# Aster32/GAN-DANet

Measured on AMD Instinct MI355X. Metric: train samples/sec (G+D step) on 256x256 tiles, higher is better.
Workload: dtype bf16; 1 GPU; full G+D train step, 8ch 256x256 -> 1024x1024 tiles, batch 32/GPU (global 32), perceptual=on, SSIM evaluated, AdamW x2; survey_config=3, per_gpu_batch=32, global_batch=32, tile=256, parallelism=dp1

## Files before the change

gan-danet_amd/_lib.py:

```python
from __future__ import annotations

import ctypes as C
import os

HERE = os.path.dirname(os.path.abspath(__file__))
LIB_PATH = os.path.join(HERE, "lib", "libgandanet_hip.so")

PREC_FP32, PREC_BF16, PREC_X3 = 0, 1, 2
PAM_BWD_K64_ATOMIC, PAM_BWD_K64_PARTS, PAM_BWD_K32_PARTS, PAM_BWD_TWO_KERNEL = 0, 1, 2, 3
ACT_NONE, ACT_RELU, ACT_LEAKY02, ACT_SIGMOID = 0, 1, 2, 3
EVAL_F64, EVAL_SKIP_NAN = 1, 2
GUARD_SQNORM, GUARD_NORM, GUARD_COEF, GUARD_OK, GUARD_APPLIED, GUARD_SKIPPED, GUARD_RECORD = range(7)
GUARD_CHUNK = 65536
FILTER_F32, FILTER_F64 = 0, 1
EDGE_REFLECT, EDGE_INTERIOR = 0, 1
FILTER_MAX_RADIUS, SAVGOL_MAX_WINDOW = 64, 33
ZOOM_MIRROR, ZOOM_NEAREST = 0, 1
FREQ_MAX_BINS, FREQ_MAX_TABLE_BYTES = 33, 16 << 20
ZONE_MAX, ZONE_EDGE_CHUNK = 32, 512
STL_MAX_T = 2048

c_fp = C.c_void_p


# ... 100 lines not shown
    "gd_pam_wide_bwd": (_i, [_p, _p, _p, _p, _p, _p, _p, _i, _i, _i, _i, _i, _i, _i, _p, _p, _p, _p, _sz, _p]),
    "gd_pam_f32_fwd": (_i, [_p, _l, _p, _l, _p, _l, _i, _i, _i, _i, _i, _p, _p, _l, _p, _l, _p, _p, _p]),
    "gd_pam_f32_bwd": (_i, [_p, _l, _p, _l, _p, _l, _p, _l, _p, _p, _i, _i, _i, _i, _i, _p, _p, _p, _p]),
    "gd_pam_attn_stats": (_i, [_p, _l, _p, _l, _i, _i, _i, _i, _f, _p, _p, _p, _p]),
    "gd_pam_attn_received": (_i, [_p, _l, _p, _l, _p, _i, _i, _i, _i, _f, _p, _p]),
    "gd_pam_attn_rows": (_i, [_p, _l, _p, _l, _p, _i, _i, _i, _i, _i, _f, _p, _p, _p]),
    "gd_round_to_16": (_i, [_p, _p, _l, _f, _i, _p]),
    "gd_chan_dot": (_i, [_p, _l, _p, _l, _i, _i, _i, _p, _p, _p, _p]),
    "gd_pam_f16_scale": (_i, [_p, _l, _i, _i, _i, _p, _p, _p, _p, _p]),
    "gd_conv3x3_nhwc_pack": (_i, [_p, _i, _i, _i, _p, _sz, _p]),
    "gd_conv3x3_nhwc": (_i, [_p, _p, _p, _p, _p, _p, _i, _i, _i, _i, _i, _i, _i, _p]),
    "gd_conv3x3_nhwc_f32out": (_i, [_p, _p, _p, _p, _l, _i, _i, _i, _i, _i, _i, _p]),
    "gd_disc_stem_fwd": (_i, [_p, _i, _i, _i, _i, _p, _p, _i, _f, _p, _i, _p]),
    "gd_disc_stem_wgrad": (_i, [_p, _p, _i, _i, _i, _i, _i, _p, _p, _i, _p]),
    "gd_disc_stem_wgrad_ws": (_i, [_p, _p, _i, _i, _i, _i, _i, _p, _p, _i, _p, _p, _sz]),
    "gd_disc_stem_dgrad": (_i, [_p, _i, _i, _i, _i, _p, _i, _p, _i, _p]),
    "gd_conv3x3_nhwc_s2": (_i, [_p, _p, _p, _p, _i, _i, _i, _i, _i, _i, _f, _i, _p]),
    "gd_conv3x3_nhwc_s2_dgrad": (_i, [_p, _p, _p, _f, _p, _i, _i, _i, _i, _i, _i, _p]),
    "gd_nhwc_flatten_fwd": (_i, [_p, _i, _i, _i, _p, _i, _p]),
    "gd_nhwc_flatten_bwd": (_i, [_p, _p, _f, _i, _i, _i, _p, _i, _p]),
    "gd_nhwc_to_nchw16": (_i, [_p, _i, _i, _i, _p, _p, _i, _p]),
    "gd_nhwc_to_nchw16_ws": (_i, [_p, _i, _i, _i, _p, _p, _i, _p, _p, _sz]),
    "gd_nhwc_stem_fwd": (_i, [_p, _i, _i, _i, _i, _p, _p, _i, _i, _p, _i, _p]),
    "gd_nhwc_stem_bwd": (_i, [_p, _i, _i, _i, _i, _p, _i, _p, _i, _p]),
    "gd_nhwc_maxpool2_fwd": (_i, [_p, _i, _i, _i, _i, _p, _i, _p]),
    "gd_nhwc_maxpool2_bwd": (_i, [_p, _p, _i, _i, _i, _i, _i, _p, _i, _p]),
    "gd_nhwc_l1": (_i, [_p, _p, _l, _p, _i, _p, _i, _p]),
    "gd_nhwc_l1_grad": (_i, [_p, _p, _l, _p, _i, _p, _i, _p]),
    "gd_shift_sum9_fwd": (_i, [_p, _p, _p, _i, _i, _i, _p]),
    "gd_shift_sum9_bwd": (_i, [_p, _p, _i, _i, _i, _p]),
    "gd_combine_inputs": (_i, [_p, _i, _i, _i, _f, _p, _i, _i, _i, _f, _p, _i, _i, _i, _p]),
    "gd_hist_match_ws_bytes": (_sz, [_l, _l]),
    "gd_hist_match": (_i, [_p, _p, _i, _l, _l, C.c_double, _p, _p, _sz, _p]),
    "gd_eval_stats_ws_bytes": (_sz, [_l]),
    "gd_eval_stats": (_i, [_p, _p, _l, _l, _p, C.c_double, C.c_double, _i, _p, _p, _sz, _p]),
    "gd_masked_plane_mean_ws_bytes": (_sz, [_l, _l]),
    "gd_masked_plane_mean": (_i, [_p, _l, _l, _p, _p, _p, _p, _sz, _p]),
    "gd_ensemble_stats": (_i, [_p, _i, _l, _l, _i, _p, _p, _p]),
    "gd_eval_merge_host": (_i, [C.POINTER(C.c_double), _l, C.POINTER(C.c_double), C.POINTER(C.c_double)]),
    "gd_grad_sqnorm_ws_bytes": (_sz, [_l]),
    "gd_grad_sqnorm": (_i, [C.POINTER(_p), C.POINTER(_l), _i, _f, _i, _p, _p, _sz, _p]),
    "gd_guard_finalize": (_i, [_p, C.c_double, _i, _p]),
    "gd_adamw_guarded": (_i, [_p, _p, _p, _p, _p, _l, _p, _f, _f, _f, _f, _f, _f, _f, _p]),
    "gd_gaussian_weights_host": (_i, [C.c_double, C.c_double, C.POINTER(C.c_double), _i]),
    "gd_correlate1d_axis": (_i, [_p, _p, _i, _l, _l, _l, C.POINTER(C.c_double), _i, _i, _p]),
    "gd_savgol_edges_axis": (_i, [_p, _p, _i, _l, _l, _l, _p, _i, _p]),
    "gd_median_nd": (_i, [_p, _p, _i, C.POINTER(C.c_int64), C.POINTER(_i), _p]),
    "gd_fill_prepare": (_i, [_p, C.c_double, _p, _p, _i, _l, _p]),
    "gd_fill_ratio": (_i, [_p, _p, _p, C.c_double, _p, _i, _l, _p]),
    "gd_zoom_axis_ws_bytes": (_sz, [_l, _l, _l, _i, _i]),
    "gd_zoom_axis": (_i, [_p, _p, _i, _i, _l, _l, _l, _l, _i, _i, _p, _sz, _p]),
    "gd_spline_prefilter_axis": (_i, [_p, _p, _i, _l, _l, _l, _p]),
    "gd_restore_units": (_i, [_p, _i, _p, _i, _p, _l, _l, C.c_double, C.c_double, C.c_double, _p, _i, _p]),
    "gd_masked_plane_mean_f64_ws_bytes": (_sz, [_l, _l]),
    "gd_masked_plane_mean_f64": (_i, [_p, _l, _l, _p, _p, _p, _p, _sz, _p]),
    "gd_blend_region": (_i, [_p, _p, _p, _i, _i, _i, _i, _i, _i, _i, _p]),
    "gd_channel_moments_ws_bytes": (_sz, [_l, _l]),
    "gd_channel_moments": (_i, [_p, _i, _l, _l, _p, _p, _sz, _p]),
    "gd_scale_from_moments_host": (_i, [C.POINTER(C.c_double), _l, C.POINTER(C.c_double), C.POINTER(C.c_double),
                                        C.POINTER(C.c_double)]),
    "gd_channel_affine": (_i, [_p, _i, _p, _i, _l, _l, _p, _p, _i, _l, _l, _p]),
    "gd_freq_cos_table_host": (_i, [_l, _i, C.POINTER(C.c_double)]),
    "gd_freq_augment_axis": (_i, [_p, _p, _i, _l, _l, _l, _p, _i, _p, _p]),
    "gd_zone_rasterize": (_i, [_p, _l, C.POINTER(_l), _i, _p, _l, _p, _l, _p, _p]),
    "gd_zone_rasterize_host": (_i, [C.POINTER(C.c_double), _l, C.POINTER(_l), _i, C.POINTER(C.c_double), _l, C.POINTER(C.c_double), _l,
                                    C.POINTER(C.c_uint32)]),
    "gd_zone_mean_ws_bytes": (_sz, [_l, _l, _i]),
    "gd_zone_mean": (_i, [_p, _i, _l, _l, _p, _i, _p, _p, _p, _p, _sz, _p]),
    "gd_stl_decompose": (_i, [_p, _i, _l, _l, _i, _i, _i, _i, _i, _i, _i, _i, _i, _p, _p, _p, _p, _p]),
    "gd_stl_decompose_host": (_i, [_p, _i, _l, _l, _i, _i, _i, _i, _i, _i, _i, _i, _i, _p, _p, _p, _p]),
    "gd_augment_d4": (_i, [_p, _p, _i, _i, _i, _i, _p, _p, _f, _p]),
    "gd_bcast_mul": (_i, [_p, _p, _p, _i, _i, _l, _i, _p]),
    "gd_row_dot": (_i, [_p, _p, _p, _l, _l, _p]),
    "gd_chan_maxmean_fwd": (_i, [_p, _p, _p, _i, _i, _l, _p]),
    "gd_chan_maxmean_bwd": (_i, [_p, _p, _p, _i, _i, _l, _p]),
    "gd_comm_unique_id": (_i, [C.c_char_p]),
    "gd_comm_init": (_i, [_i, _i, C.c_char_p]),
    "gd_comm_world": (_i, []),
    "gd_allreduce": (_i, [_p, _sz, _i, _p]),
    "gd_reduce_scatter": (_i, [_p, _p, _sz, _i, _p]),
    "gd_allgather": (_i, [_p, _p, _sz, _i, _p]),
    "gd_comm_destroy": (_i, []),
    "gd_pack_bf16": (_i, [_p, _l, _i, _i, _i, _p, _f, _p, _i, _i, _p, _i, _i, _i, _i, _p]),
    "gd_pack_16": (_i, [_p, _l, _i, _i, _i, _p, _f, _p, _i, _i, _p, _i, _i, _i, _i, _i, _p]),
    "gd_pack_16_affine": (_i, [_p, _l, _i, _i, _i, _p, _p, _i, _p, _i, _i, _p, _i, _i, _i, _p]),
}

_lib = None


class GandanetError(RuntimeError):
    pass


def load() -> C.CDLL:
    global _lib
    if _lib is not None:
        return _lib
    if not os.path.exists(LIB_PATH):
        raise GandanetError(
            f"{LIB_PATH} is missing: the HIP extension is not built (run __graft_entry__.build()). "
            "There is no CPU fallback.")
    lib = C.CDLL(LIB_PATH)
    for name, (res, args) in SIGNATURES.items():
        fn = getattr(lib, name)
        fn.restype = res
        fn.argtypes = args
    if lib.gd_sizeof_conv_desc() != C.sizeof(ConvDesc) or lib.gd_sizeof_gemm_nt_desc() != C.sizeof(GemmNTDesc):
        raise GandanetError("descriptor struct layout differs between _lib.py and libgandanet_hip.so")
    _lib = lib
    return lib


def last_error() -> str:
    buf = C.create_string_buffer(512)
    load().gd_last_error(buf, 512)
    return buf.value.decode()


def check(rc: int, what: str = "") -> None:
    if rc != 0:
        raise GandanetError(f"{what or 'gandanet call'} failed (rc={rc}): {last_error()}")
```

gan-danet_amd/csrc/gemm_conv.hip:

```cpp
#include <stdlib.h>

#include <type_traits>

#include "common.h"
#include "tile_mma.h"
#include "../../include/gandanet.h"

namespace {

using gd::TILE_BK;
using gd::TILE_BN;
constexpr int BN = TILE_BN;
constexpr int BK = TILE_BK;

template <int BM, int MODE>
__global__ __launch_bounds__(256) void conv_nn_kernel(const gd_conv_desc d) {
    constexpr bool BF16 = MODE != gd::MODE_F32;
    constexpr bool X3 = MODE == gd::MODE_X3;
    using P = gd::TilePol<MODE>;
    using elem = typename P::elem;
    constexpr int LD = P::LD;
    constexpr int WAVES_N = gd::TileGeom<BM>::WAVES_N;
    constexpr int TM = gd::TileGeom<BM>::TM;
    constexpr int TN = gd::TileGeom<BM>::TN;
// ... 400 lines not shown
                            mma(acc[sb][i][j], fa[1][i], fb[0][j]);
                            mma(acc[sb][i][j], fa[0][i], fb[1][j]);
                        }
                        mma(acc[sb][i][j], fa[0][i], fb[0][j]);
                    }
            }
        }
        } else {
#pragma unroll
        for (int ks = 0; ks < BK / 16; ++ks) {
            bf16x8_t fa[TM];
#pragma unroll
            for (int i = 0; i < TM; ++i)
                fa[i] = *reinterpret_cast<const bf16x8_t*>(As + (wm * TM * 32 + i * 32 + r) * LDA + ks * 16 + 8 * h);
#pragma unroll
            for (int sb = 0; sb < NS; ++sb) {
                bf16x8_t fb[TN];
#pragma unroll
                for (int j = 0; j < TN; ++j) {
                    const unsigned short* p = Xs + sb * (BK * XLD) + (ks * 16 + 8 * h + tq) * XLD + (wn * TN + j) * 32 + 16 * tg + 4 * tp;
                    const s16x4_t lo = __builtin_amdgcn_ds_read_tr16_b64_v4i16((__attribute__((address_space(3))) s16x4_t*)p);
                    const s16x4_t hi = __builtin_amdgcn_ds_read_tr16_b64_v4i16(
                        (__attribute__((address_space(3))) s16x4_t*)(p + 4 * XLD));
                    fb[j] = bf16x8_t{lo.x, lo.y, lo.z, lo.w, hi.x, hi.y, hi.z, hi.w};
                }
#pragma unroll
                for (int i = 0; i < TM; ++i)
#pragma unroll
                    for (int j = 0; j < TN; ++j)
                        acc[sb][i][j] = __builtin_amdgcn_mfma_f32_32x32x16_bf16(
                            __builtin_bit_cast(gd::bf16x8_native_t, fa[i]), __builtin_bit_cast(gd::bf16x8_native_t, fb[j]),
                            acc[sb][i][j], 0, 0, 0);
            }
        }
        }
    };

    load_tile(0);
    store_tile();
    __syncthreads();
    for (int t = 0; t < T; ++t) {
        if (t + 1 < T) load_tile(t + 1);
        compute_tile();
        __syncthreads();
        if (t + 1 < T) {
            store_tile();
            __syncthreads();
        }
    }

    const float alpha = d.alpha ? *d.alpha : 1.f;
#pragma unroll
    for (int sb = 0; sb < NS; ++sb)
#pragma unroll
    for (int i = 0; i < TM; ++i)
#pragma unroll
        for (int j = 0; j < TN; ++j) {
            const int pn = n0 + sb * BN + wn * TN * 32 + j * 32 + r;
            if (pn >= HW) continue;
            float rsv[16], oldv[16];
#pragma unroll
            for (int e = 0; e < 16; ++e) {
                const int m = m0 + wm * TM * 32 + i * 32 + gd::acc_row(e, h);
                rsv[e] = (d.res && m < d.M) ? d.res[(long)b * d.res_bs + (long)m * HW + pn] : 0.f;
            }
#pragma unroll
            for (int e = 0; e < 16; ++e) {
                const int m = m0 + wm * TM * 32 + i * 32 + gd::acc_row(e, h);
                oldv[e] = (d.accumulate && m < d.M) ? reinterpret_cast<const float*>(d.y)[(long)b * d.y_bs + (long)m * HW + pn] : 0.f;
            }
#pragma unroll
            for (int e = 0; e < 16; ++e) {
                const int m = m0 + wm * TM * 32 + i * 32 + gd::acc_row(e, h);
                if (m >= d.M) continue;
                float v = acc[sb][i][j][e] * alpha + rsv[e];
                if (d.bias) v += d.bias[m];
                if (d.act == GD_ACT_RELU) v = fmaxf(v, 0.f);
                else if (d.act == GD_ACT_LEAKY02) v = v >= 0.f ? v : 0.2f * v;
                reinterpret_cast<float*>(d.y)[(long)b * d.y_bs + (long)m * HW + pn] = v + oldv[e];
            }
        }
}

template <int BM, bool X3 = false>
__global__ __launch_bounds__(256) void conv1x1_tr_plain_kernel(const gd_conv_desc d) {
    constexpr int LDA = BK + 8;
    constexpr int A_PL = BM * LDA, X_PL = BK * XLD;
    constexpr int WAVES_N = gd::TileGeom<BM>::WAVES_N;
    constexpr int TM = gd::TileGeom<BM>::TM;
    constexpr int TN = gd::TileGeom<BM>::TN;
    constexpr int KPT_A = BM / 8;
    __shared__ __attribute__((aligned(16))) unsigned short As[(X3 ? 2 : 1) * BM * LDA];
    __shared__ __attribute__((aligned(16))) unsigned short Xs[(X3 ? 2 : 1) * BK * XLD];

    const int tid = threadIdx.x, lane = tid & 63, wave = tid >> 6;
    const int r = lane & 31, h = lane >> 5;
    const int wm = wave / WAVES_N, wn = wave % WAVES_N;
    const int b = blockIdx.z, m0 = blockIdx.y * BM, n0 = blockIdx.x * BN;
    const int HW = d.Ho * d.Wo;

    const int am = tid % BM, akg = tid / BM;
    const bool a_row_ok = (m0 + am) < d.M;
    const float* a_row = d.a + (long)b * d.a_bs + (long)(m0 + am) * d.a_sm;

    const int xq = tid & 31, xr0 = tid >> 5;
    const float* x_img = d.x + (long)b * d.x_bs;
    const int pq = n0 + xq * 4;
    const bool q_full = pq + 3 < HW;

    f32x16_t acc[TM][TN];
#pragma unroll
    for (int i = 0; i < TM; ++i)
#pragma unroll
        for (int j = 0; j < TN; ++j)
#pragma unroll
            for (int e = 0; e < 16; ++e) acc[i][j][e] = 0.f;

    float ra[KPT_A];
    float4 rx[4];
    const int T = (d.Ck + BK - 1) / BK;
    auto load_tile = [&](int t) {
        const int c0 = t * BK;
#pragma unroll
        for (int i = 0; i < KPT_A; ++i) {
            const int c = c0 + akg * KPT_A + i;
            ra[i] = (a_row_ok && c < d.Ck) ? a_row[(long)c * d.a_sc] : 0.f;
        }
#pragma unroll
        for (int i = 0; i < 4; ++i) {
            const int c = c0 + xr0 + 8 * i;
            float4 v = make_float4(0.f, 0.f, 0.f, 0.f);
            if (c < d.Ck) {
                const float* p = x_img + (long)c * HW + pq;
                if (q_full) {
                    v = *reinterpret_cast<const float4*>(p);
                } else {
                    if (pq + 0 < HW) v.x = p[0];
                    if (pq + 1 < HW) v.y = p[1];
                    if (pq + 2 < HW) v.z = p[2];
                }
                if (d.in_scale) {
                    const float sc = d.in_scale[c], sh = d.in_shift[c];
                    v.x = fmaf(v.x, sc, sh); v.y = fmaf(v.y, sc, sh); v.z = fmaf(v.z, sc, sh); v.w = fmaf(v.w, sc, sh);
                    if (d.in_relu) {
                        v.x = fmaxf(v.x, 0.f); v.y = fmaxf(v.y, 0.f); v.z = fmaxf(v.z, 0.f); v.w = fmaxf(v.w, 0.f);
                    }
                    if (!q_full) {
                        if (pq + 0 >= HW) v.x = 0.f;
                        if (pq + 1 >= HW) v.y = 0.f;
                        if (pq + 2 >= HW) v.z = 0.f;
                        v.w = 0.f;
                    }
                }
            }
            rx[i] = v;
        }
    };
    auto store_tile = [&]() {
        unsigned short* ap = As + am * LDA + akg * KPT_A;
        if constexpr (X3) {
#pragma unroll
            for (int i = 0; i < KPT_A; i += 4) {
                uint2 whi, wlo;
                gd_split_bf2(ra[i + 0], ra[i + 1], whi.x, wlo.x);
                gd_split_bf2(ra[i + 2], ra[i + 3], whi.y, wlo.y);
                *reinterpret_cast<uint2*>(ap + i) = whi;
                *reinterpret_cast<uint2*>(ap + A_PL + i) = wlo;
            }
#pragma unroll
            for (int i = 0; i < 4; ++i) {
                uint2 whi, wlo;
                gd_split_bf2(rx[i].x, rx[i].y, whi.x, wlo.x);
                gd_split_bf2(rx[i].z, rx[i].w, whi.y, wlo.y);
                *reinterpret_cast<uint2*>(Xs + (xr0 + 8 * i) * XLD + xq * 4) = whi;
                *reinterpret_cast<uint2*>(Xs + X_PL + (xr0 + 8 * i) * XLD + xq * 4) = wlo;
            }
            return;
        }
        if constexpr (KPT_A >= 8) {
#pragma unroll
            for (int i = 0; i < KPT_A; i += 8) {
                uint4 w;
                w.x = gd_pack_bf2(ra[i + 0], ra[i + 1]);
                w.y = gd_pack_bf2(ra[i + 2], ra[i + 3]);
                w.z = gd_pack_bf2(ra[i + 4], ra[i + 5]);
                w.w = gd_pack_bf2(ra[i + 6], ra[i + 7]);
                *reinterpret_cast<uint4*>(ap + i) = w;
            }
        } else {
            uint2 w;
            w.x = gd_pack_bf2(ra[0], ra[1]);
            w.y = gd_pack_bf2(ra[2], ra[3]);
            *reinterpret_cast<uint2*>(ap) = w;
        }
#pragma unroll
        for (int i = 0; i < 4; ++i) {
            uint2 w;
            w.x = gd_pack_bf2(rx[i].x, rx[i].y);
            w.y = gd_pack_bf2(rx[i].z, rx[i].w);
            *reinterpret_cast<uint2*>(Xs + (xr0 + 8 * i) * XLD + xq * 4) = w;
        }
    };
    const int li = lane & 15, tq = li >> 2, tp = li & 3, tg = (lane >> 4) & 1;
    auto compute_tile = [&]() {
        if constexpr (X3) {
#pragma unroll
            for (int ks = 0; ks < BK / 16; ++ks) {
                bf16x8_t fa[2][TM], fb[2][TN];
#pragma unroll
                for (int pl = 0; pl < 2; ++pl) {
#pragma unroll
                    for (int i = 0; i < TM; ++i)
                        fa[pl][i] = *reinterpret_cast<const bf16x8_t*>(As + pl * A_PL + (wm * TM * 32 + i * 32 + r) * LDA + ks * 16 + 8 * h);
#pragma unroll
                    for (int j = 0; j < TN; ++j) {
                        const unsigned short* p = Xs + pl * X_PL + (ks * 16 + 8 * h + tq) * XLD + (wn * TN + j) * 32 + 16 * tg + 4 * tp;
// ... 63 lines not shown
            if (pn >= HW) continue;
            float rsv[16], oldv[16];
#pragma unroll
            for (int e = 0; e < 16; ++e) {
                const int m = m0 + wm * TM * 32 + i * 32 + gd::acc_row(e, h);
                rsv[e] = (d.res && m < d.M) ? d.res[(long)b * d.res_bs + (long)m * HW + pn] : 0.f;
            }
#pragma unroll
            for (int e = 0; e < 16; ++e) {
                const int m = m0 + wm * TM * 32 + i * 32 + gd::acc_row(e, h);
                oldv[e] = (d.accumulate && m < d.M) ? reinterpret_cast<const float*>(d.y)[(long)b * d.y_bs + (long)m * HW + pn] : 0.f;
            }
#pragma unroll
            for (int e = 0; e < 16; ++e) {
                const int m = m0 + wm * TM * 32 + i * 32 + gd::acc_row(e, h);
                if (m >= d.M) continue;
                float v = acc[i][j][e] * alpha + rsv[e];
                if (d.bias) v += d.bias[m];
                if (d.act == GD_ACT_RELU) v = fmaxf(v, 0.f);
                else if (d.act == GD_ACT_LEAKY02) v = v >= 0.f ? v : 0.2f * v;
                reinterpret_cast<float*>(d.y)[(long)b * d.y_bs + (long)m * HW + pn] = v + oldv[e];
            }
        }
}

static bool conv1x1_tr_eligible(const gd_conv_desc& d) {
    const long HW = (long)d.Ho * d.Wo;
    return d.ks == 1 && d.stride == 1 && d.pad == 0 && (d.precision == GD_PREC_BF16 || d.precision == GD_PREC_X3) && d.out_layout == 0 && !d.out_bf16 &&
           (d.Mstore == 0 || d.Mstore == d.M) && d.Hi == d.Ho && d.Wi == d.Wo && HW % 4 == 0 && d.x_bs % 4 == 0 &&
           ((uintptr_t)d.x % 16) == 0;
}

template <int BM>
int launch(const gd_conv_desc& d, hipStream_t s) {
    const int sstep = d.sub_step > 1 ? d.sub_step : 1;
    const long hs = (d.Ho - d.sub_oy + sstep - 1) / sstep, ws = (d.Wo - d.sub_ox + sstep - 1) / sstep;
    if (hs <= 0 || ws <= 0) return 0;
    dim3 grid(gd_cdiv(hs * ws, BN), gd_cdiv(d.Mstore, BM), d.B);
    if (d.precision == GD_PREC_BF16)
        hipLaunchKernelGGL((conv_nn_kernel<BM, gd::MODE_BF16>), grid, dim3(256), 0, s, d);
    else if (d.precision == GD_PREC_X3)
        hipLaunchKernelGGL((conv_nn_kernel<BM, gd::MODE_X3>), grid, dim3(256), 0, s, d);
    else
        hipLaunchKernelGGL((conv_nn_kernel<BM, gd::MODE_F32>), grid, dim3(256), 0, s, d);
    GD_LAUNCH_CHECK();
    return 0;
}

}

extern "C" int gd_conv2d(const gd_conv_desc* dp, void* stream) {
    GD_CHECK_ARG(dp != nullptr, "gd_conv2d: null descriptor");
    gd_conv_desc d = *dp;
    if (d.Mstore < d.M) d.Mstore = d.M;
    GD_CHECK_ARG(d.B > 0 && d.M > 0 && d.Ck > 0 && d.ks > 0 && d.stride > 0 && d.pad >= 0, "gd_conv2d: bad sizes");
    GD_CHECK_ARG(d.Hi > 0 && d.Wi > 0 && d.Ho > 0 && d.Wo > 0, "gd_conv2d: bad spatial sizes");
    GD_CHECK_ARG(d.a && d.x && d.y, "gd_conv2d: null tensor");
    GD_CHECK_ARG((d.in_scale == nullptr) == (d.in_shift == nullptr), "gd_conv2d: in_scale/in_shift must come together");
    GD_CHECK_ARG(d.precision == GD_PREC_FP32 || d.precision == GD_PREC_BF16 || d.precision == GD_PREC_X3, "gd_conv2d: bad precision");
    GD_CHECK_ARG(d.out_layout == 0 || (d.out_layout == 1 && d.ldo >= d.Mstore), "gd_conv2d: bad output layout");
    GD_CHECK_ARG(!(d.out_bf16 && d.accumulate), "gd_conv2d: accumulate needs an fp32 output");
    GD_CHECK_ARG((long)d.Ho * d.Wo < (1L << 31) && d.B <= 65535, "gd_conv2d: image too large for one launch");
    GD_CHECK_ARG(d.sub_step >= 0 && d.sub_oy >= 0 && d.sub_ox >= 0 && (d.sub_step > 1 || (d.sub_oy == 0 && d.sub_ox == 0)),
                 "gd_conv2d: bad output sub-lattice");
    if (!d.transposed) {
        GD_CHECK_ARG((d.Hi + 2 * d.pad - d.ks) / d.stride + 1 == d.Ho && (d.Wi + 2 * d.pad - d.ks) / d.stride + 1 == d.Wo,
                     "gd_conv2d: Ho/Wo do not match Hi/Wi, ks, stride, pad");
    } else {
        GD_CHECK_ARG((d.Ho + 2 * d.pad - d.ks) / d.stride + 1 == d.Hi && (d.Wo + 2 * d.pad - d.ks) / d.stride + 1 == d.Wi,
                     "gd_conv2d: transposed geometry mismatch");
    }
    hipStream_t s = (hipStream_t)stream;
    static const int tr_env = getenv("GD_CONV1X1_TR") ? atoi(getenv("GD_CONV1X1_TR")) : 1;
    if (tr_env && conv1x1_tr_eligible(d)) {
        const int bm = d.M <= 32 ? 32 : (d.M <= 64 || (d.M % 128 != 0 && d.M % 128 <= 64)) ? 64 : 128;
        static const int ns_env = getenv("GD_CONV1X1_NS") ? atoi(getenv("GD_CONV1X1_NS")) : 1;
        const long HWl = (long)d.Ho * d.Wo;
        int ns = (HWl * d.B >= (1L << 18) && d.precision == GD_PREC_BF16) ? ns_env : 1;
        if (bm == 128 && ns > 2) ns = 2;
        if (ns != 1 && ns != 2 && ns != 4) ns = 1;
        dim3 grid(gd_cdiv(HWl, BN * ns), gd_cdiv(d.M, bm), d.B);
#define GD_C1X1(BM_, NS_) hipLaunchKernelGGL((conv1x1_tr_kernel<BM_, NS_>), grid, dim3(256), 0, s, d)
        if (d.precision == GD_PREC_X3) {
            if (bm == 32) hipLaunchKernelGGL((conv1x1_tr_plain_kernel<32, true>), grid, dim3(256), 0, s, d);
            else if (bm == 64) hipLaunchKernelGGL((conv1x1_tr_plain_kernel<64, true>), grid, dim3(256), 0, s, d);
            else hipLaunchKernelGGL((conv1x1_tr_plain_kernel<128, true>), grid, dim3(256), 0, s, d);
        } else if (ns == 1) {
            if (bm == 32) hipLaunchKernelGGL((conv1x1_tr_plain_kernel<32>), grid, dim3(256), 0, s, d);
            else if (bm == 64) hipLaunchKernelGGL((conv1x1_tr_plain_kernel<64>), grid, dim3(256), 0, s, d);
            else hipLaunchKernelGGL((conv1x1_tr_plain_kernel<128>), grid, dim3(256), 0, s, d);
        } else
        if (bm == 32) { if (ns == 4) GD_C1X1(32, 4); else if (ns == 2) GD_C1X1(32, 2); else GD_C1X1(32, 1); }
        else if (bm == 64) { if (ns == 4) GD_C1X1(64, 4); else if (ns == 2) GD_C1X1(64, 2); else GD_C1X1(64, 1); }
        else { if (ns == 2) GD_C1X1(128, 2); else GD_C1X1(128, 1); }
#undef GD_C1X1
        GD_LAUNCH_CHECK();
        return 0;
    }
    auto run = [&](const gd_conv_desc& dd) -> int {
        if (dd.Mstore <= 32) return launch<32>(dd, s);
        if (dd.Mstore <= 64 || (dd.Mstore % 128 != 0 && dd.Mstore % 128 <= 64)) return launch<64>(dd, s);
        return launch<128>(dd, s);
    };
    if (d.transposed && d.stride > 1 && d.sub_step <= 1) {
        for (int py = 0; py < d.stride; ++py)
            for (int px = 0; px < d.stride; ++px) {
                gd_conv_desc dd = d;
                dd.sub_oy = py; dd.sub_ox = px; dd.sub_step = d.stride;
                const int rc = run(dd);
                if (rc) return rc;
            }
        return 0;
    }
    return run(d);
}
```

gan-danet_amd/csrc/gemm_nt.hip:

```cpp
#include "common.h"
#include "tile_mma.h"
#include "../../include/gandanet.h"

namespace {

using gd::TILE_BK;
using gd::TILE_BN;
constexpr int BN = TILE_BN;
constexpr int BK = TILE_BK;

__global__ void fill_zero_kernel(float* c, long c_bs, long ldc, int B, int M, int N) {
    const long total = (long)B * M * N;
    for (long i = (long)blockIdx.x * blockDim.x + threadIdx.x; i < total; i += (long)gridDim.x * blockDim.x) {
        const int n = (int)(i % N);
        const long t = i / N;
        const int m = (int)(t % M);
        const int b = (int)(t / M);
        c[(long)b * c_bs + (long)m * ldc + n] = 0.f;
    }
}

template <int BM, int MODE, bool VEC = false>
__global__ __launch_bounds__(256) void gemm_nt_kernel(const gd_gemm_nt_desc d, int ktiles, int tiles_per_split,
                                                      int splits, float* part) {
    constexpr bool BF16 = MODE != gd::MODE_F32;
    constexpr bool X3 = MODE == gd::MODE_X3;
    constexpr int A_PL = BM * gd::TilePol<MODE>::LD, B_PL = gd::TILE_BN * gd::TilePol<MODE>::LD;
    using P = gd::TilePol<MODE>;
    using elem = typename P::elem;
    constexpr int LD = P::LD;
    constexpr int WAVES_N = gd::TileGeom<BM>::WAVES_N;
    constexpr int TM = gd::TileGeom<BM>::TM;
    constexpr int TN = gd::TileGeom<BM>::TN;
    constexpr int RA = BM / 8;
    constexpr int RB = BN / 8;

    __shared__ __attribute__((aligned(16))) elem As[P::PLANES * BM * LD];
    __shared__ __attribute__((aligned(16))) elem Bs[P::PLANES * BN * LD];

    const int tid = threadIdx.x;
    const int lane = tid & 63, wave = tid >> 6;
    const int r = lane & 31, h = lane >> 5;
    const int wm = wave / WAVES_N, wn = wave % WAVES_N;
    const int b = blockIdx.z / splits;
    const int split = blockIdx.z - b * splits;
    const int m0 = blockIdx.y * BM;
    const int n0 = blockIdx.x * BN;
    const long K = (long)d.kseg * d.klen;

    const int kk = tid & 31;
    const int r0 = tid >> 5;

    const float* a_base = d.a + (long)b * d.a_bs;
    const float* b_base = d.bm + (long)b * d.b_bs;

    int rc_off[RB];
    int rc_dydx[RB];
    const int kss = d.ks * d.ks;
    if (d.im2col) {
#pragma unroll
        for (int i = 0; i < RB; ++i) {
            const int n = n0 + r0 + 8 * i;
            if (n < d.N) {
                const int c = n / kss, tap = n - c * kss;
                const int kh = tap / d.ks, kw = tap - kh * d.ks;
                rc_off[i] = c;
                rc_dydx[i] = (kh << 16) | kw;
            } else {
                rc_off[i] = 0;
                rc_dydx[i] = -1;
            }
        }
    }
    const long HiWi = (long)d.Hi * d.Wi;

    f32x16_t acc[TM][TN];
#pragma unroll
    for (int i = 0; i < TM; ++i)
#pragma unroll
        for (int j = 0; j < TN; ++j)
#pragma unroll
            for (int e = 0; e < 16; ++e) acc[i][j][e] = 0.f;

    float ra[RA], rb[RB];
    constexpr int RAV = BM / 32, RBV = BN / 32;
    float4 va[VEC ? RAV : 1], vb[VEC ? RBV : 1];
    const int kq = tid & 7, r0v = tid >> 3;

    auto load_tile_vec = [&](int t) {
        const long k = (long)t * BK + kq * 4;
        const bool k_ok = k < K;
        const int s = k_ok ? (int)(k / d.klen) : 0;
        const long kr = k_ok ? k - (long)s * d.klen : 0;
        const float* ap = a_base + (long)s * d.a_ss + kr;
        const float* bp = b_base + (long)s * d.b_ss + kr;
#pragma unroll
        for (int i = 0; i < RAV; ++i) {
            const int m = m0 + r0v + 32 * i;
            va[i] = (k_ok && m < d.M) ? *reinterpret_cast<const float4*>(ap + (long)m * d.lda) : make_float4(0, 0, 0, 0);
        }
#pragma unroll
        for (int i = 0; i < RBV; ++i) {
            const int n = n0 + r0v + 32 * i;
            vb[i] = (k_ok && n < d.N) ? *reinterpret_cast<const float4*>(bp + (long)n * d.ldb) : make_float4(0, 0, 0, 0);
        }
    };
    auto store_tile_vec = [&]() {
#pragma unroll
        for (int i = 0; i < RAV; ++i) {
            if constexpr (X3) {
                uint2 whi, wlo;
                gd_split_bf2(va[i].x, va[i].y, whi.x, wlo.x);
                gd_split_bf2(va[i].z, va[i].w, whi.y, wlo.y);
                *reinterpret_cast<uint2*>(As + (r0v + 32 * i) * LD + kq * 4) = whi;
                *reinterpret_cast<uint2*>(As + A_PL + (r0v + 32 * i) * LD + kq * 4) = wlo;
            } else if constexpr (BF16) {
                uint2 w;
                w.x = gd_pack_bf2(va[i].x, va[i].y);
                w.y = gd_pack_bf2(va[i].z, va[i].w);
                *reinterpret_cast<uint2*>(As + (r0v + 32 * i) * LD + kq * 4) = w;
            } else {
                float* p = reinterpret_cast<float*>(As) + (r0v + 32 * i) * LD + kq * 4;
                p[0] = va[i].x; p[1] = va[i].y; p[2] = va[i].z; p[3] = va[i].w;
            }
        }
#pragma unroll
        for (int i = 0; i < RBV; ++i) {
            if (d.in_scale) {
                const int n = n0 + r0v + 32 * i;
                if (n < d.N) {
// ... 71 lines not shown
    };

    auto store_tile = [&]() {
#pragma unroll
        for (int i = 0; i < RA; ++i) {
            if constexpr (X3) gd_split_bf(ra[i], As[(r0 + 8 * i) * LD + kk], As[A_PL + (r0 + 8 * i) * LD + kk]);
            else if constexpr (BF16) As[(r0 + 8 * i) * LD + kk] = gd_f2bf(ra[i]);
            else As[(r0 + 8 * i) * LD + kk] = ra[i];
        }
#pragma unroll
        for (int i = 0; i < RB; ++i) {
            if constexpr (X3) gd_split_bf(rb[i], Bs[(r0 + 8 * i) * LD + kk], Bs[B_PL + (r0 + 8 * i) * LD + kk]);
            else if constexpr (BF16) Bs[(r0 + 8 * i) * LD + kk] = gd_f2bf(rb[i]);
            else Bs[(r0 + 8 * i) * LD + kk] = rb[i];
        }
    };

    const int t_begin = split * tiles_per_split;
    const int t_end = min(ktiles, t_begin + tiles_per_split);
    if (t_begin >= t_end) return;

    if constexpr (VEC) {
        load_tile_vec(t_begin);
        store_tile_vec();
    } else {
        load_tile(t_begin);
        store_tile();
    }
    __syncthreads();
    for (int t = t_begin; t < t_end; ++t) {
        if (t + 1 < t_end) {
            if constexpr (VEC) load_tile_vec(t + 1);
            else load_tile(t + 1);
        }
        gd::tile_mma<BM, MODE>(As, Bs, wm, wn, r, h, acc);
        __syncthreads();
        if (t + 1 < t_end) {
            if constexpr (VEC) store_tile_vec();
            else store_tile();
            __syncthreads();
        }
    }

    const float alpha = d.alpha ? *d.alpha : 1.f;
    if (part) {
        float* pb = part + ((long)split * d.B + b) * d.M * d.N;
#pragma unroll
        for (int i = 0; i < TM; ++i) {
#pragma unroll
            for (int j = 0; j < TN; ++j) {
                const int n = n0 + wn * TN * 32 + j * 32 + r;
                if (n >= d.N) continue;
#pragma unroll
                for (int e = 0; e < 16; ++e) {
                    const int m = m0 + wm * TM * 32 + i * 32 + gd::acc_row(e, h);
                    if (m < d.M) pb[(long)m * d.N + n] = acc[i][j][e] * alpha;
                }
            }
        }
        return;
    }
    float* cb = d.c + (long)b * d.c_bs;
#pragma unroll
    for (int i = 0; i < TM; ++i) {
#pragma unroll
        for (int j = 0; j < TN; ++j) {
            const int n = n0 + wn * TN * 32 + j * 32 + r;
            if (n >= d.N) continue;
            const float bias = (d.bias && split == 0) ? d.bias[n] : 0.f;
#pragma unroll
            for (int e = 0; e < 16; ++e) {
                const int m = m0 + wm * TM * 32 + i * 32 + gd::acc_row(e, h);
                if (m >= d.M) continue;
                const float v = acc[i][j][e] * alpha + bias;
                float* cp = cb + (long)m * d.ldc + n;
                if (splits > 1) atomicAdd(cp, v);
                else if (d.accumulate) *cp += v;
                else *cp = v;
            }
        }
    }
}

template <int BM>
int launch(const gd_gemm_nt_desc& d, int ktiles, int tps, int splits, float* part, hipStream_t s) {
    if (splits > 1 && !d.accumulate && !part) {
        const long total = (long)d.B * d.M * d.N;
        const int blocks = (int)((total + 255) / 256 > 4096 ? 4096 : (total + 255) / 256);
        hipLaunchKernelGGL(fill_zero_kernel, dim3(blocks), dim3(256), 0, s, d.c, d.c_bs, d.ldc, d.B, d.M, d.N);
    }
    dim3 grid(gd_cdiv(d.N, BN), gd_cdiv(d.M, BM), d.B * splits);
    const bool vec = !d.im2col && d.klen % BK == 0 && d.lda % 4 == 0 && d.ldb % 4 == 0 &&
                     d.a_ss % 4 == 0 && d.b_ss % 4 == 0 && d.a_bs % 4 == 0 && d.b_bs % 4 == 0 &&
                     ((uintptr_t)d.a % 16) == 0 && ((uintptr_t)d.bm % 16) == 0;
    if (d.precision == GD_PREC_BF16) {
        if (vec) hipLaunchKernelGGL((gemm_nt_kernel<BM, gd::MODE_BF16, true>), grid, dim3(256), 0, s, d, ktiles, tps, splits, part);
        else hipLaunchKernelGGL((gemm_nt_kernel<BM, gd::MODE_BF16, false>), grid, dim3(256), 0, s, d, ktiles, tps, splits, part);
    } else if (d.precision == GD_PREC_X3) {
        if (vec) hipLaunchKernelGGL((gemm_nt_kernel<BM, gd::MODE_X3, true>), grid, dim3(256), 0, s, d, ktiles, tps, splits, part);
        else hipLaunchKernelGGL((gemm_nt_kernel<BM, gd::MODE_X3, false>), grid, dim3(256), 0, s, d, ktiles, tps, splits, part);
    } else {
        if (vec) hipLaunchKernelGGL((gemm_nt_kernel<BM, gd::MODE_F32, true>), grid, dim3(256), 0, s, d, ktiles, tps, splits, part);
        else hipLaunchKernelGGL((gemm_nt_kernel<BM, gd::MODE_F32, false>), grid, dim3(256), 0, s, d, ktiles, tps, splits, part);
    }
    GD_LAUNCH_CHECK();
    if (part) return gd_det_reduce_launch(part, splits, d.c, d.B, d.M, d.N, d.c_bs, d.ldc, d.bias, d.accumulate, s);
    return 0;
}

struct NtPlan { int ktiles, bm, tiles_per_split, splits, ordered; size_t ws_needed; };
int nt_plan(const gd_gemm_nt_desc& d, size_t ws_bytes, NtPlan* p) {
    GD_CHECK_ARG(d.B > 0 && d.M > 0 && d.N > 0 && d.kseg > 0 && d.klen > 0, "gd_gemm_nt: bad sizes");
    GD_CHECK_ARG((long)d.kseg * d.klen < (1L << 31), "gd_gemm_nt: reduction too long");
    GD_CHECK_ARG((d.in_scale == nullptr) == (d.in_shift == nullptr), "gd_gemm_nt: in_scale/in_shift must come together");
    GD_CHECK_ARG(d.precision == GD_PREC_FP32 || d.precision == GD_PREC_BF16 || d.precision == GD_PREC_X3, "gd_gemm_nt: bad precision");
    if (d.im2col) {
        GD_CHECK_ARG(d.ks > 0 && d.stride > 0 && d.pad >= 0 && d.Hi > 0 && d.Wi > 0 && d.Ho > 0 && d.Wo > 0,
                     "gd_gemm_nt: bad im2col geometry");
        GD_CHECK_ARG(d.klen == (long)d.Ho * d.Wo, "gd_gemm_nt: im2col needs klen == Ho*Wo");
        GD_CHECK_ARG(d.N % (d.ks * d.ks) == 0, "gd_gemm_nt: im2col needs N == C*ks*ks");
        GD_CHECK_ARG((d.Hi + 2 * d.pad - d.ks) / d.stride + 1 == d.Ho && (d.Wi + 2 * d.pad - d.ks) / d.stride + 1 == d.Wo,
                     "gd_gemm_nt: im2col Ho/Wo mismatch");
    }
    GD_CHECK_ARG((long)d.B * 4096 < 65535L * 64, "gd_gemm_nt: batch too large");
    const int ktiles = gd_cdiv((long)d.kseg * d.klen, BK);
    const int bm = d.M <= 32 ? 32 : (d.M <= 64 || (d.M % 128 != 0 && d.M % 128 <= 64)) ? 64 : 128;
    int splits = d.splits;
    if (splits <= 0) {
        const long tiles = (long)gd_cdiv(d.N, BN) * gd_cdiv(d.M, bm) * d.B;
        splits = (int)(2048 / tiles);
        if (splits < 1) splits = 1;
        if (splits > ktiles / 8) splits = ktiles / 8 > 0 ? ktiles / 8 : 1;
    }
    if (splits > ktiles) splits = ktiles;
    const bool det = gd_get_deterministic() != 0, ordered_mode = det && gd_get_det_reduce() == 1;
    if (det && !ordered_mode) splits = 1;
    if ((long)d.B * splits > 65535) splits = (int)(65535 / d.B);
    const size_t out_bytes = (size_t)d.B * d.M * d.N * sizeof(float);
    if (ordered_mode) {
        const size_t fit = ws_bytes / out_bytes;
        if ((size_t)splits > fit) splits = (int)fit;
        if (splits < 2) splits = 1;
    }
    const int tps = (ktiles + splits - 1) / splits;
    splits = (ktiles + tps - 1) / tps;
    p->ktiles = ktiles; p->bm = bm; p->tiles_per_split = tps; p->splits = splits;
    p->ordered = ordered_mode && splits > 1;
    p->ws_needed = p->ordered ? (size_t)splits * out_bytes : 0;
    return 0;
}

}

extern "C" int gd_gemm_nt_plan(const gd_gemm_nt_desc* dp, size_t ws_bytes, int* splits, size_t* ws_needed) {
    GD_CHECK_ARG(dp != nullptr, "gd_gemm_nt_plan: null descriptor");
    NtPlan p;
    if (nt_plan(*dp, ws_bytes, &p)) return -1;
    if (splits) *splits = p.splits;
    if (ws_needed) *ws_needed = p.ws_needed;
    return 0;
}

extern "C" int gd_gemm_nt_ws(const gd_gemm_nt_desc* dp, void* stream, void* ws, size_t ws_bytes) {
    GD_CHECK_ARG(dp != nullptr, "gd_gemm_nt: null descriptor");
    const gd_gemm_nt_desc& d = *dp;
    GD_CHECK_ARG(d.a && d.bm && d.c, "gd_gemm_nt: null tensor");
    GD_CHECK_ARG(((uintptr_t)ws % 16) == 0, "gd_gemm_nt: the workspace must be 16-byte aligned");
    NtPlan p;
    if (nt_plan(d, ws ? ws_bytes : 0, &p)) return -1;
    float* part = p.ordered ? (float*)ws : nullptr;
    hipStream_t s = (hipStream_t)stream;
    if (p.bm == 32) return launch<32>(d, p.ktiles, p.tiles_per_split, p.splits, part, s);
    if (p.bm == 64) return launch<64>(d, p.ktiles, p.tiles_per_split, p.splits, part, s);
    return launch<128>(d, p.ktiles, p.tiles_per_split, p.splits, part, s);
}

extern "C" int gd_gemm_nt(const gd_gemm_nt_desc* dp, void* stream) { return gd_gemm_nt_ws(dp, stream, nullptr, 0); }
```

gan-danet_amd/csrc/pointwise.hip:

```cpp
#include "common.h"
#include "../../include/gandanet.h"

#include <math.h>

namespace {

constexpr int RED_BLOCKS = 1024;

static inline int grid_for(long n, int per_block = 256 * 4) {
    long g = (n + per_block - 1) / per_block;
    if (g < 1) g = 1;
    if (g > 8192) g = 8192;
    return (int)g;
}

__device__ __forceinline__ float act_f(float v, int act) {
    if (act == GD_ACT_RELU) return fmaxf(v, 0.f);
    if (act == GD_ACT_LEAKY02) return v >= 0.f ? v : 0.2f * v;
    if (act == GD_ACT_SIGMOID) return 1.f / (1.f + __expf(-v));
    return v;
}

__global__ void act_fwd_kernel(const float* __restrict__ x, float* __restrict__ y, long n, int act) {
    for (long i = (long)blockIdx.x * blockDim.x + threadIdx.x; i < n; i += (long)gridDim.x * blockDim.x)
// ... 377 lines not shown
        for (long j = threadIdx.x; j < n; j += 256) s = fmaf(ap[j], bp[j], s);
        s = gd_block_sum(s, red);
        if (threadIdx.x == 0) out[row] = s;
    }
}
__global__ void chan_maxmean_fwd_kernel(const float* __restrict__ x, float* __restrict__ y, int* __restrict__ idx, int C,
                                        long HW, long total) {
    for (long i = (long)blockIdx.x * blockDim.x + threadIdx.x; i < total; i += (long)gridDim.x * blockDim.x) {
        const long b = i / HW, p = i - b * HW;
        const float* xp = x + b * C * HW + p;
        float mx = xp[0], sum = xp[0];
        int am = 0;
        for (int c = 1; c < C; ++c) {
            const float v = xp[(long)c * HW];
            sum += v;
            if (v > mx) { mx = v; am = c; }
        }
        y[b * 2 * HW + p] = mx;
        y[b * 2 * HW + HW + p] = sum / (float)C;
        idx[i] = am;
    }
}
__global__ void chan_maxmean_bwd_kernel(const float* __restrict__ dy, const int* __restrict__ idx, float* __restrict__ dx,
                                        int C, long HW, long total) {
    const float inv_c = 1.f / (float)C;
    for (long i = (long)blockIdx.x * blockDim.x + threadIdx.x; i < total; i += (long)gridDim.x * blockDim.x) {
        const long bc = i / HW, p = i - bc * HW;
        const long b = bc / C;
        const int c = (int)(bc - b * C);
        const float gmax = dy[b * 2 * HW + p], gmean = dy[b * 2 * HW + HW + p];
        dx[i] = gmean * inv_c + (idx[b * HW + p] == c ? gmax : 0.f);
    }
}

__global__ __launch_bounds__(256) void chan_dot_kernel(const float* __restrict__ a, long a_bs, const float* __restrict__ o,
                                                      long o_bs, int C, int N, const float* __restrict__ gamma,
                                                      float* __restrict__ draw, float* __restrict__ delta) {
    const int b = blockIdx.y;
    const int i = blockIdx.x * 256 + threadIdx.x;
    if (i >= N) return;
    const float* ap = a + (long)b * a_bs + i;
    const float* op = o + (long)b * o_bs + i;
    float s = 0.f;
    for (int c = 0; c < C; ++c) s = fmaf(ap[(long)c * N], op[(long)c * N], s);
    draw[(long)b * N + i] = s;
    delta[(long)b * N + i] = s * (*gamma);
}

__global__ __launch_bounds__(256) void absmax_kernel(const float* __restrict__ a, long a_bs, long chw, float* __restrict__ ws) {
    __shared__ float red[8];
    const float* ap = a + (long)blockIdx.y * a_bs;
    float m = 0.f;
    for (long i = (long)blockIdx.x * 256 + threadIdx.x; i < chw; i += (long)gridDim.x * 256) {
        const float v = fabsf(ap[i]);
        m = v > m ? v : m;
    }
    m = gd_block_max(m, red);
    if (threadIdx.x == 0) ws[blockIdx.y * gridDim.x + blockIdx.x] = m;
}
__global__ __launch_bounds__(256) void f16_scale_kernel(const float* __restrict__ ws, int nparts, const float* __restrict__ gamma,
                                                       float* __restrict__ delta, long n, float* __restrict__ scales) {
    __shared__ float red[8];
    __shared__ float s_up;
    float m = 0.f;
    for (int i = threadIdx.x; i < nparts; i += 256) m = fmaxf(m, ws[i]);
    m = gd_block_max(m, red);
    if (threadIdx.x == 0) {
        const float g = *gamma;
        const float t = m * fabsf(g);
        int e = 0;
        if (t > 0.f && t < 3.0e38f) frexpf(t, &e);
        e = e > 100 ? 100 : (e < -100 ? -100 : e);
        s_up = ldexpf(1.f, -e);
        if (blockIdx.x == 0) {
            scales[0] = g * s_up;
            scales[1] = ldexpf(1.f, e);
        }
    }
    __syncthreads();
    const float up = s_up;
    for (long i = (long)blockIdx.x * 256 + threadIdx.x; i < n; i += (long)gridDim.x * 256) delta[i] *= up;
}

__global__ __launch_bounds__(256) void bce_kernel(const float* __restrict__ z, long n, float label, float inv_n,
                                                 float* __restrict__ dz, float* __restrict__ ws) {
    __shared__ float red[8];
    float s = 0.f;
    for (long i = (long)blockIdx.x * 256 + threadIdx.x; i < n; i += (long)gridDim.x * 256) {
        const float v = z[i];
        s += fmaxf(v, 0.f) - v * label + log1pf(expf(-fabsf(v)));
        if (dz) dz[i] = (1.f / (1.f + expf(-v)) - label) * inv_n;
    }
    s = gd_block_sum(s, red);
    if (threadIdx.x == 0) ws[blockIdx.x] = s;
}
__global__ __launch_bounds__(256) void bce_target_kernel(const float* __restrict__ z, const float* __restrict__ t, long n,
                                                        float inv_n, float* __restrict__ dz, float* __restrict__ dt,
                                                        float* __restrict__ ws) {
    __shared__ float red[8];
    float s = 0.f;
    for (long i = (long)blockIdx.x * 256 + threadIdx.x; i < n; i += (long)gridDim.x * 256) {
        const float v = z[i], y = t[i];
        s += fmaxf(v, 0.f) - v * y + log1pf(expf(-fabsf(v)));
        if (dz) dz[i] = (1.f / (1.f + expf(-v)) - y) * inv_n;
        if (dt) dt[i] = -v * inv_n;
    }
    s = gd_block_sum(s, red);
    if (threadIdx.x == 0) ws[blockIdx.x] = s;
}
__global__ void leaky_fwd_kernel(const float* __restrict__ x, float* __restrict__ y, long n, float slope) {
    for (long i = (long)blockIdx.x * blockDim.x + threadIdx.x; i < n; i += (long)gridDim.x * blockDim.x) {
        const float v = x[i];
        y[i] = v >= 0.f ? v : slope * v;
    }
}
__global__ void leaky_bwd_kernel(const float* __restrict__ x, const float* __restrict__ dy, float* __restrict__ dx, long n,
                                 float slope) {
    for (long i = (long)blockIdx.x * blockDim.x + threadIdx.x; i < n; i += (long)gridDim.x * blockDim.x)
        dx[i] = x[i] >= 0.f ? dy[i] : slope * dy[i];
}
template <bool L1>
__global__ __launch_bounds__(256) void diff_loss_kernel(const float* __restrict__ a, const float* __restrict__ b, long n,
                                                       float inv_n, float* __restrict__ da, float* __restrict__ ws) {
    __shared__ float red[8];
    float s = 0.f;
    for (long i = (long)blockIdx.x * 256 + threadIdx.x; i < n; i += (long)gridDim.x * 256) {
        const float dv = a[i] - b[i];
        if (L1) {
            s += fabsf(dv);
            if (da) da[i] = dv > 0.f ? inv_n : (dv < 0.f ? -inv_n : 0.f);
        } else {
            s = fmaf(dv, dv, s);
            if (da) da[i] = 2.f * dv * inv_n;
        }
    }
    s = gd_block_sum(s, red);
    if (threadIdx.x == 0) ws[blockIdx.x] = s;
}
__global__ __launch_bounds__(256) void tv_kernel(const float* __restrict__ x, long planes, int H, int W, float kh, float kw,
                                                float* __restrict__ dx, float* __restrict__ ws_h, float* __restrict__ ws_w) {
    __shared__ float red[8];
    const long total = planes * H * W;
    float sh = 0.f, sw = 0.f;
    for (long i = (long)blockIdx.x * 256 + threadIdx.x; i < total; i += (long)gridDim.x * 256) {
        const int xx = (int)(i % W);
        const int yy = (int)((i / W) % H);
        const float v = x[i];
        float g = 0.f;
        if (yy + 1 < H) { const float d = x[i + W] - v; sh = fmaf(d, d, sh); g -= 2.f * kh * d; }
        if (yy > 0) { const float d = v - x[i - W]; g += 2.f * kh * d; }
        if (xx + 1 < W) { const float d = x[i + 1] - v; sw = fmaf(d, d, sw); g -= 2.f * kw * d; }
        if (xx > 0) { const float d = v - x[i - 1]; g += 2.f * kw * d; }
        if (dx) dx[i] = g;
    }
    sh = gd_block_sum(sh, red);
    sw = gd_block_sum(sw, red);
    if (threadIdx.x == 0) { ws_h[blockIdx.x] = sh; ws_w[blockIdx.x] = sw; }
}
__global__ __launch_bounds__(256) void tv_final_kernel(const float* __restrict__ ws_h, const float* __restrict__ ws_w,
                                                      int nparts, float kh, float kw, float* __restrict__ out) {
    __shared__ double redd[8];
    double a = 0, b = 0;
    for (int i = threadIdx.x; i < nparts; i += 256) { a += ws_h[i]; b += ws_w[i]; }
    a = gd_wave_sum_d(a);
    b = gd_wave_sum_d(b);
    if ((threadIdx.x & 63) == 0) { redd[threadIdx.x >> 6] = a; redd[4 + (threadIdx.x >> 6)] = b; }
// ... 283 lines not shown
    GD_LAUNCH_CHECK();
    return 0;
}
extern "C" int gd_pack_16_split(const float* s, long s_bs, int B, int R, int Cc, const float* row_scale, const float* row_shift,
                                int relu, void* plain, long p_bs, int ldp, long p_cs, int p_ncopy, int p_pattern, void* tr,
                                long t_bs, int ldt, long t_cs, int t_ncopy, int t_pattern, void* stream) {
    return gd_pack_16_split_masked(s, s_bs, B, R, Cc, row_scale, row_shift, relu, plain, p_bs, ldp, p_cs, p_ncopy, p_pattern, tr,
                                   t_bs, ldt, t_cs, t_ncopy, t_pattern, nullptr, 0, stream);
}
extern "C" int gd_split3_weights(const float* w, long A, long Bn, long Cn, float* out, void* stream) {
    GD_CHECK_ARG(w && out && A > 0 && Bn > 0 && Cn > 0, "gd_split3_weights: bad arguments");
    const long total = A * Bn * Cn;
    hipLaunchKernelGGL(split3_weights_kernel, dim3(grid_for(total) > 4096 ? 4096 : grid_for(total)), dim3(256), 0, GD_S, w, A, Bn, Cn, out);
    GD_LAUNCH_CHECK();
    return 0;
}
extern "C" int gd_pack_bf16(const float* s, long s_bs, int B, int R, int Cc, const float* scale_dev, float scale_imm,
                            void* plain, int Rp_plain, int ld_plain, void* transposed, int Ccp_t, int ld_t, int perm16,
                            int ones_row, void* stream) {
    return gd_pack_16(s, s_bs, B, R, Cc, scale_dev, scale_imm, plain, Rp_plain, ld_plain, transposed, Ccp_t, ld_t, perm16,
                      ones_row, 0, stream);
}
extern "C" int gd_augment_d4(const float* src, float* dst, int B, int C, int H, int W, const int* ops, const float* noise,
                             float noise_scale, void* stream) {
    GD_CHECK_ARG(src && dst && ops && src != dst && B > 0 && C > 0 && H > 0 && W > 0, "gd_augment_d4: bad arguments");
    const long total = (long)B * C * H * W;
    hipLaunchKernelGGL(augment_d4_kernel, dim3(grid_for(total)), dim3(256), 0, GD_S, src, dst, C, H, W, ops, noise,
                       noise_scale, total);
    GD_LAUNCH_CHECK();
    return 0;
}
extern "C" int gd_bcast_mul(const float* x, const float* att, float* y, int B, int C, long HW, int mode, void* stream) {
    GD_CHECK_ARG(x && att && y && B > 0 && C > 0 && HW > 0 && (mode == 0 || mode == 1), "gd_bcast_mul: bad arguments");
    const long total = (long)B * C * HW;
    hipLaunchKernelGGL(bcast_mul_kernel, dim3(grid_for(total)), dim3(256), 0, GD_S, x, att, y, C, HW, mode, total);
    GD_LAUNCH_CHECK();
    return 0;
}
extern "C" int gd_row_dot(const float* a, const float* b, float* out, long rows, long n, void* stream) {
    GD_CHECK_ARG(a && b && out && rows > 0 && n > 0, "gd_row_dot: bad arguments");
    hipLaunchKernelGGL(row_dot_kernel, dim3((unsigned)(rows < 8192 ? rows : 8192)), dim3(256), 0, GD_S, a, b, out, rows, n);
    GD_LAUNCH_CHECK();
    return 0;
}
extern "C" int gd_chan_maxmean_fwd(const float* x, float* y, int* idx, int B, int C, long HW, void* stream) {
    GD_CHECK_ARG(x && y && idx && B > 0 && C > 0 && HW > 0, "gd_chan_maxmean_fwd: bad arguments");
    const long total = (long)B * HW;
    hipLaunchKernelGGL(chan_maxmean_fwd_kernel, dim3(grid_for(total, 256)), dim3(256), 0, GD_S, x, y, idx, C, HW, total);
    GD_LAUNCH_CHECK();
    return 0;
}
extern "C" int gd_chan_maxmean_bwd(const float* dy, const int* idx, float* dx, int B, int C, long HW, void* stream) {
    GD_CHECK_ARG(dy && idx && dx && B > 0 && C > 0 && HW > 0, "gd_chan_maxmean_bwd: bad arguments");
    const long total = (long)B * C * HW;
    hipLaunchKernelGGL(chan_maxmean_bwd_kernel, dim3(grid_for(total)), dim3(256), 0, GD_S, dy, idx, dx, C, HW, total);
    GD_LAUNCH_CHECK();
    return 0;
}
extern "C" int gd_chan_dot(const float* a, long a_bs, const float* o, long o_bs, int B, int C, int N, const float* gamma,
                           float* d_raw, float* delta, void* stream) {
    GD_CHECK_ARG(a && o && gamma && d_raw && delta && B > 0 && B <= 65535 && C > 0 && N > 0, "gd_chan_dot: bad arguments");
    hipLaunchKernelGGL(chan_dot_kernel, dim3(gd_cdiv(N, 256), B), dim3(256), 0, GD_S, a, a_bs, o, o_bs, C, N, gamma, d_raw,
                       delta);
    GD_LAUNCH_CHECK();
    return 0;
}

extern "C" int gd_pam_f16_scale(const float* dout, long dout_bs, int B, int C, int N, const float* gamma, float* delta,
                                float* scales, float* ws, void* stream) {
    GD_CHECK_ARG(dout && gamma && delta && scales && ws && B > 0 && B <= 65535 && C > 0 && N > 0, "gd_pam_f16_scale: bad arguments");
    const long chw = (long)C * N;
    int g = grid_for(chw);
    g = g > RED_BLOCKS / B ? RED_BLOCKS / B : g;
    g = g < 1 ? 1 : g;
    GD_CHECK_ARG((long)g * B <= RED_BLOCKS, "gd_pam_f16_scale: batch larger than the reduction workspace (1024 parts)");
    hipLaunchKernelGGL(absmax_kernel, dim3(g, B), dim3(256), 0, GD_S, dout, dout_bs, chw, ws);
    const long n = (long)B * N;
    hipLaunchKernelGGL(f16_scale_kernel, dim3(grid_for(n) > 256 ? 256 : grid_for(n)), dim3(256), 0, GD_S, ws, g * B, gamma, delta, n,
                       scales);
    GD_LAUNCH_CHECK();
    return 0;
}

extern "C" int gd_bce_logits(const float* z, long n, float label, float* out, float* dz, float* ws, void* stream) {
    GD_CHECK_ARG(z && out && ws && n > 0, "gd_bce_logits: bad arguments");
    const int g = grid_for(n) > RED_BLOCKS ? RED_BLOCKS : grid_for(n);
    hipLaunchKernelGGL(bce_kernel, dim3(g), dim3(256), 0, GD_S, z, n, label, 1.f / (float)n, dz, ws);
    hipLaunchKernelGGL(reduce_final_kernel, dim3(1), dim3(256), 0, GD_S, ws, g, 1.f / (float)n, out, 0);
    GD_LAUNCH_CHECK();
    return 0;
}
extern "C" int gd_bce_logits_target(const float* z, const float* t, long n, float* out, float* dz, float* dt, float* ws,
                                    void* stream) {
    GD_CHECK_ARG(z && t && out && ws && n > 0, "gd_bce_logits_target: bad arguments");
    const int g = grid_for(n) > RED_BLOCKS ? RED_BLOCKS : grid_for(n);
    hipLaunchKernelGGL(bce_target_kernel, dim3(g), dim3(256), 0, GD_S, z, t, n, 1.f / (float)n, dz, dt, ws);
    hipLaunchKernelGGL(reduce_final_kernel, dim3(1), dim3(256), 0, GD_S, ws, g, 1.f / (float)n, out, 0);
    GD_LAUNCH_CHECK();
    return 0;
}
extern "C" int gd_leaky_fwd(const float* x, float* y, long n, float slope, void* stream) {
    GD_CHECK_ARG(x && y && n > 0, "gd_leaky_fwd: bad arguments");
    hipLaunchKernelGGL(leaky_fwd_kernel, dim3(grid_for(n)), dim3(256), 0, GD_S, x, y, n, slope);
    GD_LAUNCH_CHECK();
    return 0;
}
extern "C" int gd_leaky_bwd(const float* x, const float* dy, float* dx, long n, float slope, void* stream) {
    GD_CHECK_ARG(x && dy && dx && n > 0, "gd_leaky_bwd: bad arguments");
    hipLaunchKernelGGL(leaky_bwd_kernel, dim3(grid_for(n)), dim3(256), 0, GD_S, x, dy, dx, n, slope);
    GD_LAUNCH_CHECK();
    return 0;
}
extern "C" int gd_mse(const float* a, const float* b, long n, float* out, float* da, float* ws, void* stream) {
    GD_CHECK_ARG(a && b && out && ws && n > 0, "gd_mse: bad arguments");
    const int g = grid_for(n) > RED_BLOCKS ? RED_BLOCKS : grid_for(n);
    hipLaunchKernelGGL((diff_loss_kernel<false>), dim3(g), dim3(256), 0, GD_S, a, b, n, 1.f / (float)n, da, ws);
    hipLaunchKernelGGL(reduce_final_kernel, dim3(1), dim3(256), 0, GD_S, ws, g, 1.f / (float)n, out, 0);
    GD_LAUNCH_CHECK();
    return 0;
}
extern "C" int gd_l1(const float* a, const float* b, long n, float* out, float* da, float* ws, void* stream) {
    GD_CHECK_ARG(a && b && out && ws && n > 0, "gd_l1: bad arguments");
    const int g = grid_for(n) > RED_BLOCKS ? RED_BLOCKS : grid_for(n);
    hipLaunchKernelGGL((diff_loss_kernel<true>), dim3(g), dim3(256), 0, GD_S, a, b, n, 1.f / (float)n, da, ws);
    hipLaunchKernelGGL(reduce_final_kernel, dim3(1), dim3(256), 0, GD_S, ws, g, 1.f / (float)n, out, 0);
    GD_LAUNCH_CHECK();
    return 0;
}
extern "C" int gd_tv(const float* x, int B, int C, int H, int W, float weight, float* out, float* dx, float* ws,
                     void* stream) {
    GD_CHECK_ARG(x && out && ws && B > 0 && C > 0 && H > 1 && W > 1, "gd_tv: bad arguments");
    const long planes = (long)B * C;
    const double count_h = (double)planes * (H - 1) * W, count_w = (double)planes * H * (W - 1);
    const float kh = (float)(weight * 2.0 / count_h / B), kw = (float)(weight * 2.0 / count_w / B);
    const long n = planes * H * W;
    const int g = grid_for(n) > RED_BLOCKS ? RED_BLOCKS : grid_for(n);
    hipLaunchKernelGGL(tv_kernel, dim3(g), dim3(256), 0, GD_S, x, planes, H, W, kh, kw, dx, ws, ws + RED_BLOCKS);
    hipLaunchKernelGGL(tv_final_kernel, dim3(1), dim3(256), 0, GD_S, ws, ws + RED_BLOCKS, g, kh, kw, out);
    GD_LAUNCH_CHECK();
    return 0;
}
static int ssim_window(int window, SsimWin* win) {
    if (!(window > 0 && window <= 15 && (window & 1))) return -1;
    win->n = window;
    float tmp[16], sum = 0.f;
    for (int i = 0; i < window; ++i) {
        const float d = (float)(i - window / 2);
        tmp[i] = expf(-(d * d) / (2.f * 1.5f * 1.5f));
        sum += tmp[i];
    }
    for (int i = 0; i < 16; ++i) win->g[i] = i < window ? tmp[i] / sum : 0.f;
    return 0;
}
static int ssim_gx(int H, int W, int BC) {
    int gx = (int)(((long)H * W + 255) / 256);
    if (gx > 64) gx = 64;
    while ((long)gx * BC > 2048 && gx > 1) gx >>= 1;
    return gx;
}
extern "C" int gd_ssim(const float* a, const float* b, int BC, int H, int W, int window, float* out, float* ws,
                       void* stream) {
    GD_CHECK_ARG(a && b && out && ws && BC > 0 && H > 0 && W > 0, "gd_ssim: bad arguments");
    SsimWin win;
    GD_CHECK_ARG(ssim_window(window, &win) == 0, "gd_ssim: window must be odd and <= 15");
    const int gx = ssim_gx(H, W, BC);
    GD_CHECK_ARG((long)gx * BC <= 2048 && BC <= 65535, "gd_ssim: too many planes for the workspace");
// ... 51 lines not shown
```

gan-danet_amd/kern.py:

```python
from __future__ import annotations

import ctypes as C
import math
import os
from typing import Optional, Tuple

import torch

from . import _lib as L

Tensor = torch.Tensor


def _stream() -> int:
    return torch.cuda.current_stream().cuda_stream


def _ptr(t: Optional[Tensor]):
    return None if t is None else t.data_ptr()


def _chk(t: Tensor, name: str = "tensor", dtype=torch.float32) -> None:
    if not t.is_cuda:
        raise L.GandanetError(f"{name}: expected a GPU tensor (there is no CPU fallback in the product path)")
# ... 9 lines not shown


def _bview(t: Tensor, name: str = "tensor") -> int:
    _chk(t, name)
    if t.dim() == 4:
        b, c, h, w = t.shape
        ok = t.stride(3) == 1 and t.stride(2) == w and t.stride(1) == h * w
        inner = c * h * w
    elif t.dim() == 3:
        b, c, n = t.shape
        ok = t.stride(2) == 1 and t.stride(1) == n
        inner = c * n
    else:
        raise L.GandanetError(f"{name}: expected a 3-D or 4-D tensor")
    if not ok:
        raise L.GandanetError(f"{name}: per-image block must be dense, got strides {t.stride()}")
    bs = t.stride(0) if b > 1 else inner
    if b > 1 and bs < inner:
        raise L.GandanetError(f"{name}: overlapping batch stride")
    return bs


def lib():
    return L.load()


WGRAD_X_NHWC = os.environ.get("GD_WGRAD_X_NHWC", "1") != "0"
USE_CONV3X3_FAST = True


PROFILE_ON = False
PROFILE_CONV = os.environ.get("GD_PROFILE_CONV", "0") == "1"
PROFILE: list = []


class _Bracket:

    def __init__(self, name: str, flops: float, nbytes: float = 0.0):
        self.name, self.flops, self.nbytes = name, flops, nbytes

    def __enter__(self):
        if PROFILE_ON:
            self.e0 = torch.cuda.Event(enable_timing=True)
            self.e1 = torch.cuda.Event(enable_timing=True)
            self.e0.record()
        return self

    def __exit__(self, *exc):
        if PROFILE_ON:
            self.e1.record()
            PROFILE.append((self.name, self.e0, self.e1, self.flops, self.nbytes))
        return False


class _ConvBracket(_Bracket):

    def __init__(self, kind, k, stride, cin, cout, ho, wo, b):
        super().__init__(f"conv_{kind}_k{k}s{stride}_{cin}->{cout}@{ho}x{wo}", 2.0 * k * k * cin * cout * ho * wo * b)

    def __enter__(self):
        return super().__enter__() if PROFILE_CONV else self

    def __exit__(self, *exc):
        return super().__exit__(*exc) if PROFILE_CONV else False


def profile_summary():
    torch.cuda.synchronize()
    agg = {}
    for name, e0, e1, fl, nb in PROFILE:
        a = agg.setdefault(name, [0, 0.0, 0.0, 0.0])
        a[0] += 1
        a[1] += e0.elapsed_time(e1)
        a[2] += fl
        a[3] += nb
    return {k: (v[0], v[1] / v[0], v[2] / v[0], v[3] / v[0]) for k, v in agg.items()}


def conv_nn(*, B: int, M: int, Ck: int, ks: int, stride: int, pad: int, transposed: bool, Hi: int, Wi: int,
            Ho: int, Wo: int, a: Tensor, a_bs: int, a_sm: int, a_sc: int, a_st: int, x: Tensor, x_bs: int,
            y: Tensor, y_bs: int, precision: int, Mstore: int = 0, in_scale: Optional[Tensor] = None,
            in_shift: Optional[Tensor] = None, in_relu: bool = False, out_layout: int = 0, out_bf16: bool = False,
            ldo: int = 0, alpha: Optional[Tensor] = None, bias: Optional[Tensor] = None,
            res: Optional[Tensor] = None, res_bs: int = 0, act: int = 0, accumulate: bool = False) -> None:
    d = L.ConvDesc()
    d.B, d.M, d.Mstore, d.Ck, d.ks, d.stride, d.pad = B, M, max(M, Mstore), Ck, ks, stride, pad
    d.transposed = int(transposed)
    d.Hi, d.Wi, d.Ho, d.Wo = Hi, Wi, Ho, Wo
    d.a, d.a_bs, d.a_sm, d.a_sc, d.a_st = _ptr(a), a_bs, a_sm, a_sc, a_st
    d.x, d.x_bs = _ptr(x), x_bs
    d.in_scale, d.in_shift, d.in_relu = _ptr(in_scale), _ptr(in_shift), int(in_relu)
    d.y, d.y_bs = _ptr(y), y_bs
    d.out_layout, d.out_bf16, d.ldo = out_layout, int(out_bf16), ldo
    d.alpha, d.bias, d.res, d.res_bs = _ptr(alpha), _ptr(bias), _ptr(res), res_bs
    d.act, d.accumulate, d.precision = act, int(accumulate), precision
    if USE_CONV3X3_FAST and lib().gd_conv3x3_eligible(C.byref(d)):
        nbytes = int(lib().gd_conv3x3_ws_bytes(M, Ck))
        ws = torch.empty(nbytes // 2, device=x.device, dtype=torch.bfloat16)
        L.check(lib().gd_conv3x3(C.byref(d), _ptr(ws), nbytes, _stream()), "gd_conv3x3")
        return
    L.check(lib().gd_conv2d(C.byref(d), _stream()), "gd_conv2d")


def conv_out_size(h: int, k: int, stride: int, pad: int) -> int:
    return (h + 2 * pad - k) // stride + 1


def conv2d_fwd(x: Tensor, w: Tensor, bias: Optional[Tensor], stride: int, pad: int, precision: int, *,
               act: int = 0, out: Optional[Tensor] = None, in_scale=None, in_shift=None, in_relu=False,
               accumulate: bool = False) -> Tensor:
    xbs = _bview(x, "conv input")
    _dense(w, "conv weight")
    B, Cin, Hi, Wi = x.shape
    Cout, Cin_w, k, k2 = w.shape
    if Cin_w != Cin or k != k2:
        raise L.GandanetError(f"conv2d: weight {tuple(w.shape)} does not match input {tuple(x.shape)}")
    Ho, Wo = conv_out_size(Hi, k, stride, pad), conv_out_size(Wi, k, stride, pad)
    if out is None:
        out = torch.empty(B, Cout, Ho, Wo, device=x.device, dtype=torch.float32)
    elif tuple(out.shape) != (B, Cout, Ho, Wo):
        raise L.GandanetError("conv2d: bad out shape")
    with _ConvBracket("fwd", k, stride, Cin, Cout, Ho, Wo, B):
        conv_nn(B=B, M=Cout, Ck=Cin, ks=k, stride=stride, pad=pad, transposed=False, Hi=Hi, Wi=Wi, Ho=Ho, Wo=Wo,
                a=w, a_bs=0, a_sm=Cin * k * k, a_sc=k * k, a_st=1, x=x, x_bs=xbs, y=out, y_bs=_bview(out, "conv out"),
                precision=precision, in_scale=in_scale, in_shift=in_shift, in_relu=in_relu, bias=bias, act=act,
                accumulate=accumulate)
    return out


def conv2d_dgrad(dy: Tensor, w: Tensor, in_hw: Tuple[int, int], stride: int, pad: int, precision: int, *,
                 out: Optional[Tensor] = None, accumulate: bool = False, alpha: Optional[Tensor] = None) -> Tensor:
    dbs = _bview(dy, "conv dy")
    B, Cout, Ho, Wo = dy.shape
    Cout_w, Cin, k, _ = w.shape
    Hi, Wi = in_hw
    if Cout_w != Cout:
        raise L.GandanetError("conv2d_dgrad: weight/out-channel mismatch")
    if out is None:
        out = torch.empty(B, Cin, Hi, Wi, device=dy.device, dtype=torch.float32)
    with _ConvBracket("dgrad", k, stride, Cin, Cout, Ho, Wo, B):
        conv_nn(B=B, M=Cin, Ck=Cout, ks=k, stride=stride, pad=pad, transposed=True, Hi=Ho, Wi=Wo, Ho=Hi, Wo=Wi,
                a=w, a_bs=0, a_sm=k * k, a_sc=Cin * k * k, a_st=1, x=dy, x_bs=dbs, y=out, y_bs=_bview(out, "conv dx"),
                precision=precision, accumulate=accumulate, alpha=alpha)
    return out


def gemm_nt(*, B: int, M: int, N: int, kseg: int, klen: int, a: Tensor, a_bs: int, a_ss: int, lda: int,
            bm: Tensor, b_bs: int, b_ss: int, ldb: int, c: Tensor, c_bs: int, ldc: int, precision: int,
            im2col=None, in_scale=None, in_shift=None, in_relu=False, alpha=None, bias=None,
            accumulate: bool = False, splits: int = 0) -> None:
    d = L.GemmNTDesc()
    d.B, d.M, d.N, d.kseg, d.klen = B, M, N, kseg, klen
    d.a, d.a_bs, d.a_ss, d.lda = _ptr(a), a_bs, a_ss, lda
    d.bm, d.b_bs, d.b_ss, d.ldb = _ptr(bm), b_bs, b_ss, ldb
    if im2col is not None:
        d.im2col = 1
        d.ks, d.stride, d.pad, d.Hi, d.Wi, d.Ho, d.Wo = im2col
    d.in_scale, d.in_shift, d.in_relu = _ptr(in_scale), _ptr(in_shift), int(in_relu)
    d.c, d.c_bs, d.ldc = _ptr(c), c_bs, ldc
    d.alpha, d.bias = _ptr(alpha), _ptr(bias)
    d.accumulate, d.splits, d.precision = int(accumulate), splits, precision
    L.check(lib().gd_gemm_nt_ws(C.byref(d), _stream(), *det_ws()), "gd_gemm_nt")


def conv2d_wgrad(dy: Tensor, x: Tensor, k: int, stride: int, pad: int, precision: int, *, in_scale=None,
                 in_shift=None, in_relu=False, alpha: Optional[Tensor] = None, splits: int = 0) -> Tensor:
    if alpha is not None and not (k == 1 and stride == 1 and pad == 0):
        raise L.GandanetError("conv2d_wgrad: alpha is supported for 1x1 convs only")
    dbs, xbs = _bview(dy, "wgrad dy"), _bview(x, "wgrad x")
    B, Cout, Ho, Wo = dy.shape
    _, Cin, Hi, Wi = x.shape
    dw = torch.empty(Cout, Cin, k, k, device=dy.device, dtype=torch.float32)
    with _ConvBracket("wgrad", k, stride, Cin, Cout, Ho, Wo, B):
        return _conv2d_wgrad(dy, x, k, stride, pad, precision, in_scale, in_shift, in_relu, dw, dbs, xbs, B, Cout, Cin, Hi,
                             Wi, Ho, Wo, alpha, splits)


def _conv2d_wgrad(dy, x, k, stride, pad, precision, in_scale, in_shift, in_relu, dw, dbs, xbs, B, Cout, Cin, Hi, Wi, Ho, Wo,
# ... 432 lines not shown
              t_shape=None, perm16: bool = False, ones_row: int = -1, f16: bool = False):
    sbs = _bview(s, "pack input")
    B = s.shape[0]
    plain = tr = None
    rp = ldp = ccp = ldt = 0
    dt = torch.float16 if f16 else torch.bfloat16
    if plain_shape is not None:
        rp, ldp = plain_shape
        plain = torch.empty(B, rp, ldp, device=s.device, dtype=dt)
    if t_shape is not None:
        ccp, ldt = t_shape
        tr = torch.empty(B, ccp, ldt, device=s.device, dtype=dt)
    L.check(lib().gd_pack_16(_ptr(s), sbs, B, R, Cc, _ptr(scale), float(scale_imm), _ptr(plain), rp, ldp, _ptr(tr),
                             ccp, ldt, int(perm16), int(ones_row), int(f16), _stream()), "gd_pack_16")
    return plain, tr


def pack_nhwc16_affine(x: Tensor, scale: Optional[Tensor], shift: Optional[Tensor], relu: bool) -> Tensor:
    sbs = _bview(x, "pack input")
    B, Cn, H, W = x.shape
    out = torch.empty(B, H * W, Cn, device=x.device, dtype=torch.bfloat16)
    L.check(lib().gd_pack_16_affine(_ptr(x), sbs, B, Cn, H * W, _ptr(scale), _ptr(shift), int(relu), None, 0, 0, _ptr(out),
                                    H * W, Cn, 0, _stream()), "gd_pack_16_affine")
    return out


def augment_d4(x: Tensor, ops: Tensor, noise: Optional[Tensor] = None, noise_scale: float = 0.05) -> Tensor:
    _dense(x, "augment input")
    _chk(ops, "augment ops", torch.int32)
    B, Cn, H, W = x.shape
    if ops.numel() != B or (noise is not None and _dense(noise, "noise").shape != x.shape):
        raise L.GandanetError("augment_d4: ops must hold one word per sample and noise must match the batch")
    y = torch.empty_like(x)
    L.check(lib().gd_augment_d4(_ptr(x), _ptr(y), B, Cn, H, W, _ptr(ops), _ptr(noise), float(noise_scale), _stream()),
            "gd_augment_d4")
    return y


def bcast_mul(x: Tensor, att: Tensor, mode: int) -> Tensor:
    _dense(x), _dense(att)
    B, Cn = x.shape[0], x.shape[1]
    HW = x[0, 0].numel()
    if att.numel() != (B * Cn if mode == 0 else B * HW):
        raise L.GandanetError(f"bcast_mul: gate of {att.numel()} elements does not match x {tuple(x.shape)} (mode {mode})")
    y = torch.empty_like(x)
    L.check(lib().gd_bcast_mul(_ptr(x), _ptr(att), _ptr(y), B, Cn, HW, mode, _stream()), "gd_bcast_mul")
    return y


def row_dot(a: Tensor, b: Tensor, rows: int) -> Tensor:
    _dense(a), _dense(b)
    n = a.numel() // rows
    out = torch.empty(rows, device=a.device, dtype=torch.float32)
    L.check(lib().gd_row_dot(_ptr(a), _ptr(b), _ptr(out), rows, n, _stream()), "gd_row_dot")
    return out


def chan_maxmean_fwd(x: Tensor):
    _dense(x)
    B, Cn, H, W = x.shape
    y = torch.empty(B, 2, H, W, device=x.device, dtype=torch.float32)
    idx = torch.empty(B, H * W, device=x.device, dtype=torch.int32)
    L.check(lib().gd_chan_maxmean_fwd(_ptr(x), _ptr(y), _ptr(idx), B, Cn, H * W, _stream()), "gd_chan_maxmean_fwd")
    return y, idx


def chan_maxmean_bwd(dy: Tensor, idx: Tensor, Cn: int) -> Tensor:
    _dense(dy)
    B, _, H, W = dy.shape
    dx = torch.empty(B, Cn, H, W, device=dy.device, dtype=torch.float32)
    L.check(lib().gd_chan_maxmean_bwd(_ptr(dy), _ptr(idx), _ptr(dx), B, Cn, H * W, _stream()), "gd_chan_maxmean_bwd")
    return dx


def chan_dot(a: Tensor, o: Tensor, gamma: Tensor):
    abs_, obs = _bview(a), _bview(o)
    B, Cn = a.shape[0], a.shape[1]
    N = a[0, 0].numel()
    d_raw = torch.empty(B, N, device=a.device, dtype=torch.float32)
    delta = torch.empty_like(d_raw)
    L.check(lib().gd_chan_dot(_ptr(a), abs_, _ptr(o), obs, B, Cn, N, _ptr(gamma), _ptr(d_raw), _ptr(delta), _stream()),
            "gd_chan_dot")
    return d_raw, delta


def pam_f16_scale(dout: Tensor, gamma: Tensor, delta: Tensor) -> Tensor:
    bs = _bview(dout, "dOut")
    B, Cn = dout.shape[0], dout.shape[1]
    N = dout[0, 0].numel()
    scales = torch.empty(2, device=dout.device, dtype=torch.float32)
    L.check(lib().gd_pam_f16_scale(_ptr(dout), bs, B, Cn, N, _ptr(gamma), _ptr(_dense(delta)), _ptr(scales),
                                   _ptr(_red_ws(dout.device)), _stream()), "gd_pam_f16_scale")
    return scales


PAM_NOMAX = os.environ.get("GD_PAM_NOMAX", "1") != "0"


def pam_key_sqnorm_max(kt: Tensor, N: int, f16: bool = False) -> Tensor:
    B, Npad = kt.shape[0], kt.shape[1]
    out = torch.empty(B, device=kt.device, dtype=torch.float32)
    L.check(lib().gd_pam_key_sqnorm_max(_ptr(kt), B, N, Npad, int(f16), _ptr(out), _stream()), "gd_pam_key_sqnorm_max")
    return out


def pam_flash_fwd(qt, kt, v, B, N, Npad, Cn, Cp, gamma, x, out, o_attn, lse, r_alg: int = 32, v_ones: bool = False,
                  f16: bool = False, k_sqmax: Optional[Tensor] = None):
    with _Bracket("pam_flash_fwd", 2.0 * N * N * (r_alg + Cn) * B):
        L.check(lib().gd_pam_flash_fwd(_ptr(qt), _ptr(kt), _ptr(v), B, N, Npad, Cn, Cp, int(v_ones), int(f16),
                                       _ptr(gamma), _ptr(x), _bview(x), _ptr(out), _bview(out), _ptr(o_attn), _ptr(lse),
                                       _ptr(k_sqmax), _stream()), "gd_pam_flash_fwd")


PAM_SHIFT = os.environ.get("GD_PAM_SHIFT", "0") != "0"
PAM_SHIFT_SAMPLES = int(os.environ.get("GD_PAM_SHIFT_SAMPLES", "256"))


def pam_flash_fwd_shift(qt, kt, v, B, N, Npad, Cn, Cp, gamma, x, out, o_attn, lse, r_alg: int = 32, v_ones: bool = False,
                        nsample: Optional[int] = None, return_flags: bool = False):
    _bf(qt, "qt"), _bf(kt, "kt")
    nbytes = int(lib().gd_pam_fwd_shift_ws_bytes(B, Npad))
    ws = torch.empty(nbytes // 4, device=qt.device, dtype=torch.int32)
    with _Bracket("pam_flash_fwd", 2.0 * N * N * (r_alg + Cn) * B):
        L.check(lib().gd_pam_flash_fwd_shift(_ptr(qt), _ptr(kt), _ptr(v), B, N, Npad, Cn, Cp, int(v_ones), _ptr(gamma), _ptr(x),
                                             _bview(x), _ptr(out), _bview(out), _ptr(o_attn), _ptr(lse),
                                             int(nsample or PAM_SHIFT_SAMPLES), _ptr(ws), nbytes, _stream()),
                "gd_pam_flash_fwd_shift")
    if return_flags:
        return ws[B * Npad:].clone()
    return None


PAM_BWD_FORM = int(os.environ.get("GD_PAM_BWD", "0"))
PAM_SCRATCH_CAP = 40 << 30
DETERMINISTIC = False
DET_REDUCE = "unsplit"
_DET_REDUCE_MODES = {"unsplit": 0, "ordered": 1}
DET_WS_BYTES: Optional[int] = None
_DET_WS: dict = {}


def set_deterministic(on: bool, reduce: Optional[str] = None) -> None:
    global DETERMINISTIC, DET_REDUCE
    if reduce is not None and reduce not in _DET_REDUCE_MODES:
        raise L.GandanetError(f"set_deterministic: reduce must be one of {sorted(_DET_REDUCE_MODES)}, got {reduce!r}")
    DETERMINISTIC = bool(on)
    lib().gd_set_deterministic(int(DETERMINISTIC))
    if reduce is not None:
        L.check(lib().gd_set_det_reduce(_DET_REDUCE_MODES[reduce]), "gd_set_det_reduce")
        DET_REDUCE = reduce


def det_ws_bytes() -> int:
    return int(DET_WS_BYTES) if DET_WS_BYTES is not None else int(os.environ.get("GD_DET_WS_MB", "256")) << 20


def det_ws() -> Tuple[Optional[int], int]:
    if not (DETERMINISTIC and DET_REDUCE == "ordered"):
        return None, 0
    nbytes = det_ws_bytes()
    if nbytes <= 0:
        return None, 0
    key = (torch.cuda.current_device(), _stream())
    t = _DET_WS.get(key)
    if t is None or t.numel() != nbytes:
        t = _DET_WS[key] = torch.empty(nbytes, device=torch.device("cuda", key[0]), dtype=torch.uint8)
# ... 844 lines not shown
```

gan-danet_amd/ops.py:

```python
from __future__ import annotations

import os
from typing import List, Optional

import torch
from torch.autograd import Function

from . import _lib as L
from . import kern as K
from .config import config, operand_mode, sixteen_bit

ACT_NONE, ACT_RELU, ACT_LEAKY, ACT_SIGMOID = L.ACT_NONE, L.ACT_RELU, L.ACT_LEAKY02, L.ACT_SIGMOID


def _prec(layer: str = "other") -> int:
    mode = operand_mode(layer)
    return L.PREC_BF16 if mode == "16" else L.PREC_X3 if mode == "x3" else L.PREC_FP32


def _x3(layer: str) -> bool:
    return operand_mode(layer) == "x3"


def _x3_eligible(x, w, stride, pad, act) -> bool:
# ... 293 lines not shown
        return slab

    @staticmethod
    def backward(ctx, dslab_in):
        slab, *saved = ctx.saved_tensors
        nl, C0, g, training, prec, has_bias, packed, split, sync = ctx.cfg
        packs = saved[5 * nl:]
        B, _, H, W = slab.shape
        dslab = torch.empty(slab.shape, device=slab.device, dtype=torch.float32)
        K.copy_slab(_c(dslab_in), dslab)
        grads: List[Optional[torch.Tensor]] = [None] * (6 * nl)
        for l in reversed(range(nl)):
            scale, shift, mean, invstd, cw = saved[5 * l: 5 * l + 5]
            cl = C0 + l * g
            xin = slab[:, :cl]
            dy = dslab[:, cl:cl + g]
            if packed:
                dxt, grads[6 * l + 4] = _packed3x3_bwd(dy, packs[l], cw, H, W, split, True, True, dw_first=True)
            else:
                grads[6 * l + 4] = K.conv2d_wgrad(dy, xin, 3, 1, 1, prec, in_scale=scale, in_shift=shift, in_relu=True)
                dxt = K.conv2d_dgrad(dy, cw, (H, W), 1, 1, prec)
            if has_bias[l]:
                grads[6 * l + 5] = K.channel_sum(dy)
            dgamma, dbeta, _ = _bn_bwd(dxt, xin, scale, shift, mean, invstd, ACT_RELU, training, sync,
                                       dx=dslab[:, :cl], accumulate_dx=True)
            grads[6 * l + 0], grads[6 * l + 1] = dgamma, dbeta
        dx = torch.empty(B, C0, H, W, device=slab.device, dtype=torch.float32)
        K.copy_slab(dslab[:, :C0], dx)
        return (dx, None, None, None, *grads)


def _npad(n: int) -> int:
    return (n + 255) // 256 * 256


def _cp(c: int) -> int:
    return (c + 31) // 32 * 32


def _pam_wide(Cn: int, r: int) -> bool:
    return K.PAM_WIDE and sixteen_bit("pam") and 192 < Cn <= 511 and r <= 63


def _pam_f32(B: int, Cn: int, r: int, N: int) -> bool:
    if operand_mode("pam") != "exact" or not (1 <= Cn <= 511 and 1 <= r <= 63):
        return False
    if K.PAM_F32_FLASH is None:
        return B * N * N > K.PAM_F32_AUTO_ELEMS
    return bool(K.PAM_F32_FLASH)


def _pad_plane(t: torch.Tensor, N: int, Np: int) -> torch.Tensor:
    if N == Np:
        return t
    B, R = t.shape[0], t.shape[1]
    out = torch.zeros(B, R, Np, device=t.device, dtype=torch.float32)
    K.copy_rows(t, K._bview(t), N, out, R * Np, Np, B, R, N)
    return out


def _pam_pack16(q, k, v, r, Cn, N, D, ones_row, f16):
    Np, Cp = _npad(N), _cp(Cn)
    _, qt = K.pack_bf16(q, r, N, scale_imm=K.LOG2E, t_shape=(Np, D), f16=f16)
    kn, kt = K.pack_bf16(k, r, N, plain_shape=(D, Np), t_shape=(Np, D), perm16=True, ones_row=D - 1, f16=f16)
    vn, vt = K.pack_bf16(v, Cn, N, plain_shape=(Cp, Np), t_shape=(Np, Cp), perm16=True, ones_row=ones_row, f16=f16)
    return qt, kt, kn, vn, vt


def _pam_route(B: int, Cn: int, r: int, N: int) -> str:
    if sixteen_bit("pam") and Cn <= 192 and r <= 31:
        return "narrow"
    if _pam_wide(Cn, r):
        return "wide"
    return "f32" if _pam_f32(B, Cn, r, N) else "chain"


def _pam_forward(x, wq, bq, wk, bk, wv, bv, gamma_p, out3, prec):
    B, Cn, H, W = x.shape
    N = H * W
    r = wq.shape[0]
    x3 = x.view(B, Cn, N)
    route = _pam_route(B, Cn, r, N)
    if route != "chain" and PAM_CAT and (bq is None) == (bk is None) == (bv is None):
        wc = torch.empty(2 * r + Cn, Cn, 1, 1, device=x.device, dtype=torch.float32)
        for w_, lo in ((wq, 0), (wk, r), (wv, 2 * r)):
            K.copy_slab(_c(w_).view(1, w_.shape[0], Cn), wc.view(1, 2 * r + Cn, Cn)[:, lo:lo + w_.shape[0]])
        bc = None
        if bq is not None:
            bc = torch.empty(2 * r + Cn, device=x.device, dtype=torch.float32)
            for b_, lo in ((bq, 0), (bk, r), (bv, 2 * r)):
                K.copy_slab(b_.view(1, -1, 1), bc.view(1, -1, 1)[:, lo:lo + b_.numel()])
        y3 = K.conv2d_fwd(x, wc, bc, 1, 0, prec).view(B, 2 * r + Cn, N)
        q, k, v = y3[:, :r], y3[:, r:2 * r], y3[:, 2 * r:]
    else:
        q = K.conv2d_fwd(x, wq, bq, 1, 0, prec).view(B, r, N)
        k = K.conv2d_fwd(x, wk, bk, 1, 0, prec).view(B, r, N)
        v = K.conv2d_fwd(x, wv, bv, 1, 0, prec).view(B, Cn, N)
    if route in ("narrow", "wide"):
        Np, Cp = _npad(N), _cp(Cn)
        f16 = _pam_f16()
        D = 32 if route == "narrow" else K.pam_wide_slots(r)
        ones = Cp - 1 if route == "narrow" and Cn < Cp else -1
        qt, kt, kn, vn, vt = _pam_pack16(q, k, v, r, Cn, N, D, ones, f16)
        del q, k, v
        y3 = None
        o_attn = torch.empty(B, Cn, N, device=x.device, dtype=torch.float32)
        lse = torch.empty(B, N, device=x.device, dtype=torch.float32)
        if route == "wide":
            K.pam_wide_fwd(qt, kt, vn, B, N, Np, Cn, Cp, D, gamma_p, x3, out3, o_attn, lse, r_alg=r, f16=f16)
        elif K.PAM_SHIFT and not f16:
            K.pam_flash_fwd_shift(qt, kt, vn, B, N, Np, Cn, Cp, gamma_p, x3, out3, o_attn, lse, r_alg=r, v_ones=ones >= 0)
        else:
            k_sqmax = K.pam_key_sqnorm_max(kt, N, f16) if K.PAM_NOMAX else None
            K.pam_flash_fwd(qt, kt, vn, B, N, Np, Cn, Cp, gamma_p, x3, out3, o_attn, lse, r_alg=r, v_ones=ones >= 0, f16=f16,
                            k_sqmax=k_sqmax)
        return route, (qt, kt, kn, vt, o_attn, lse)
    if route == "f32":
        Np = _npad(N)
        q, k, v = _pad_plane(q, N, Np), _pad_plane(k, N, Np), _pad_plane(v, N, Np)
        o_attn = torch.empty(B, Cn, N, device=x.device, dtype=torch.float32)
        lse = torch.empty(B, N, device=x.device, dtype=torch.float32)
        K.pam_f32_fwd(q, k, v, B, N, Np, Cn, r, gamma_p, x3, out3, o_attn, lse)
        return route, (q, k, v, o_attn, lse)
    prec = prec if sixteen_bit("pam") else L.PREC_FP32
    return route, _pam_chain_fwd(q, k, v, x3, gamma_p, out3, prec)


def _pam_chain_fwd(q, k, v, x3, gamma_p, out3, prec):
    B, r, N = q.shape
    Cn = v.shape[1]
    qt_, kt_ = K.transpose(q), K.transpose(k)
    s = torch.empty(B, N, N, device=q.device, dtype=torch.float32)
    K.gemm_nt(B=B, M=N, N=N, kseg=1, klen=r, a=qt_, a_bs=N * r, a_ss=0, lda=r, bm=kt_, b_bs=N * r, b_ss=0,
              ldb=r, c=s, c_bs=N * N, ldc=N, precision=prec, splits=1)
    p = K.softmax_rows(s, 1.0, out=s)
    o_attn = torch.empty(B, Cn, N, device=q.device, dtype=torch.float32)
    K.gemm_nt(B=B, M=Cn, N=N, kseg=1, klen=N, a=v, a_bs=Cn * N, a_ss=0, lda=N, bm=p, b_bs=N * N, b_ss=0,
              ldb=N, c=o_attn, c_bs=Cn * N, ldc=N, precision=prec, splits=1)
    K.copy_slab(x3, out3)
    _axpy_dev3(o_attn, gamma_p, out3)
    return qt_, kt_, v, p, o_attn


def _pam_chain_bwd(pam_saved, gamma_p, d_pam, pprec):
    qt_, kt_, v, p, o_attn = pam_saved
    B, N, r = qt_.shape
    Cn = v.shape[1]
    dev = v.device
    dop = torch.empty(B, Cn, N, device=dev, dtype=torch.float32)
    K.copy_slab(d_pam, dop)
    dgamma_p = K.dot(dop, o_attn)
    K.scale_dev(dop, gamma_p, out=dop)
    dp = torch.empty(B, N, N, device=dev, dtype=torch.float32)
    K.conv_nn(B=B, M=N, Ck=Cn, ks=1, stride=1, pad=0, transposed=False, Hi=1, Wi=N, Ho=1, Wo=N, a=dop,
              a_bs=Cn * N, a_sm=1, a_sc=N, a_st=0, x=v, x_bs=Cn * N, y=dp, y_bs=N * N, precision=pprec)
    ds = K.softmax_rows_bwd(p, dp, 1.0)
    del dp
    dv = torch.empty(B, Cn, N, device=dev, dtype=torch.float32)
    K.conv_nn(B=B, M=Cn, Ck=N, ks=1, stride=1, pad=0, transposed=False, Hi=1, Wi=N, Ho=1, Wo=N, a=dop,
              a_bs=Cn * N, a_sm=N, a_sc=1, a_st=0, x=p, x_bs=N * N, y=dv, y_bs=Cn * N, precision=pprec)
    dqt = torch.empty(B, N, r, device=dev, dtype=torch.float32)
    dkt = torch.empty(B, N, r, device=dev, dtype=torch.float32)
    K.conv_nn(B=B, M=N, Ck=N, ks=1, stride=1, pad=0, transposed=False, Hi=1, Wi=r, Ho=1, Wo=r, a=ds,
              a_bs=N * N, a_sm=N, a_sc=1, a_st=0, x=kt_, x_bs=N * r, y=dqt, y_bs=N * r, precision=pprec)
    K.conv_nn(B=B, M=N, Ck=N, ks=1, stride=1, pad=0, transposed=False, Hi=1, Wi=r, Ho=1, Wo=r, a=ds,
              a_bs=N * N, a_sm=1, a_sc=N, a_st=0, x=qt_, x_bs=N * r, y=dkt, y_bs=N * r, precision=pprec)
    return K.transpose(dqt), K.transpose(dkt), dv, dgamma_p


def _pam_backward(route, pam_saved, x, wq, wk, wv, gamma_p, d_pam, dx, prec, has_bias):
    B, Cn, H, W = x.shape
    N = H * W
    r = wq.shape[0]
    if route == "f32":
        q, k, v, o_attn, lse = pam_saved
        Np = q.shape[2]
        d_raw, delta = K.chan_dot(d_pam, o_attn, gamma_p)
        dgamma_p = K.dot(d_raw, None)
        if Np == N:
            gdo = torch.empty(B, Cn, N, device=x.device, dtype=torch.float32)
            K.copy_slab(d_pam, gdo)
        else:
            gdo = _pad_plane(d_pam, N, Np)
        K.scale_dev(gdo, gamma_p, out=gdo)
        dq = torch.empty(B, r, N, device=x.device, dtype=torch.float32)
        dk = torch.empty(B, r, N, device=x.device, dtype=torch.float32)
        dv = torch.empty(B, Cn, N, device=x.device, dtype=torch.float32)
        K.pam_f32_bwd(q, k, v, gdo, lse, delta, B, N, Np, Cn, r, dq, dk, dv)
    elif route in ("narrow", "wide"):
        qt, kt, kn, vt, o_attn, lse = pam_saved
        Np, Cp = _npad(N), _cp(Cn)
        d_raw, delta = K.chan_dot(d_pam, o_attn, gamma_p)
        dgamma_p = K.dot(d_raw, None)
        f16 = qt.dtype == torch.float16
        s_up, s_inv = gamma_p, None
        if f16:
            scales = K.pam_f16_scale(d_pam, gamma_p, delta)
            s_up, s_inv = scales[0:1], scales[1:2]
        _, dot_ = K.pack_bf16(d_pam, Cn, N, scale=s_up, t_shape=(Np, Cp), f16=f16)
        if route == "wide":
            D = qt.shape[2]
            dqn = torch.empty(B, D, Np, device=x.device, dtype=torch.float32)
            dkn = torch.empty(B, D, Np, device=x.device, dtype=torch.float32)
            dvp = torch.empty(B, Cp, Np, device=x.device, dtype=torch.float32)
            K.pam_wide_bwd(qt, kt, kn, vt, dot_, lse, delta, B, N, Np, Cp, D, dqn, dkn, dvp, r_alg=r, c_alg=Cn, f16=f16)
        elif PAM_CAT and Np == N and K.pam_bwd_form() == L.PAM_BWD_K64_ATOMIC:
            R = 64 + Cp
            dcat = torch.empty(B, R, Np, device=x.device, dtype=torch.float32)
            K.pam_flash_bwd(qt, kt, kn, vt, dot_, lse, delta, B, N, Np, Cp, dcat[:, 0:32], dcat[:, 32:64], dcat[:, 64:],
                            r_alg=r, c_alg=Cn, f16=f16, out_bs=R * Np)
            wcat = torch.zeros(R, Cn, 1, 1, device=x.device, dtype=torch.float32)
            for w_, lo in ((wq, 0), (wk, 32), (wv, 64)):
                K.copy_slab(_c(w_).view(1, w_.shape[0], Cn), wcat.view(1, R, Cn)[:, lo:lo + w_.shape[0]])
            dcat4 = dcat.view(B, R, H, W)
            dwc = K.conv2d_wgrad(dcat4, x, 1, 1, 0, prec, alpha=s_inv)
            dbc = K.channel_sum(dcat4) if any(has_bias) else None
            if dbc is not None and s_inv is not None:
                K.scale_dev(dbc, s_inv, out=dbc)
            K.conv2d_dgrad(dcat4, wcat, (H, W), 1, 0, prec, out=dx.view(B, Cn, H, W), accumulate=True, alpha=s_inv)
            grads = []
            for (lo, n), hb in zip(((0, r), (32, r), (64, Cn)), has_bias):
                grads.append(dwc[lo:lo + n])
                grads.append(dbc[lo:lo + n] if hb else None)
            return (*grads, dgamma_p)
        else:
            dqn = torch.empty(B, 32, Np, device=x.device, dtype=torch.float32)
            dkn = torch.empty(B, 32, Np, device=x.device, dtype=torch.float32)
            dvp = torch.empty(B, Cp, Np, device=x.device, dtype=torch.float32)
            K.pam_flash_bwd(qt, kt, kn, vt, dot_, lse, delta, B, N, Np, Cp, dqn, dkn, dvp, r_alg=r, c_alg=Cn, f16=f16)
        if s_inv is not None:
            for t in (dqn, dkn, dvp):
                K.scale_dev(t, s_inv, out=t)
        dq, dk, dv = _compact(dqn, r, N), _compact(dkn, r, N), _compact(dvp, Cn, N)
    else:
        pprec = prec if sixteen_bit("pam") else L.PREC_FP32
        dq, dk, dv, dgamma_p = _pam_chain_bwd(pam_saved, gamma_p, d_pam, pprec)
    grads = []
    splits = 1 if route == "f32" else 0
    for dy3, w, hb in ((dq, wq, has_bias[0]), (dk, wk, has_bias[1]), (dv, wv, has_bias[2])):
        dy4 = dy3.view(B, dy3.shape[1], H, W)
        grads.append(K.conv2d_wgrad(dy4, x, 1, 1, 0, prec, splits=splits))
        grads.append(K.channel_sum(dy4) if hb else None)
        K.conv2d_dgrad(dy4, w, (H, W), 1, 0, prec, out=dx.view(B, Cn, H, W), accumulate=True)
    return (*grads, dgamma_p)


def _cam_forward(x, gamma_c, out3, prec=L.PREC_FP32):
    B, Cn, H, W = x.shape
    N = H * W
    x3 = x.view(B, Cn, N)
    e = torch.empty(B, Cn, Cn, device=x.device, dtype=torch.float32)
    K.gemm_nt(B=B, M=Cn, N=Cn, kseg=1, klen=N, a=x3, a_bs=Cn * N, a_ss=0, lda=N, bm=x3, b_bs=Cn * N, b_ss=0,
              ldb=N, c=e, c_bs=Cn * Cn, ldc=Cn, precision=L.PREC_FP32)
    att = K.softmax_rows(e, -1.0, out=e)
    K.conv_nn(B=B, M=Cn, Ck=Cn, ks=1, stride=1, pad=0, transposed=False, Hi=1, Wi=N, Ho=1, Wo=N, a=att,
              a_bs=Cn * Cn, a_sm=Cn, a_sc=1, a_st=0, x=x3, x_bs=Cn * N, y=out3, y_bs=K._bview(out3),
              precision=prec, alpha=gamma_c, res=x3, res_bs=Cn * N)
    return att


def _cam_backward(att, x, gamma_c, d_cam, dx, prec=L.PREC_FP32):
    B, Cn, H, W = x.shape
    N = H * W
    x3 = x.view(B, Cn, N)
    d_bs = K._bview(d_cam)
    da = torch.empty(B, Cn, Cn, device=x.device, dtype=torch.float32)
    K.gemm_nt(B=B, M=Cn, N=Cn, kseg=1, klen=N, a=d_cam, a_bs=d_bs, a_ss=0, lda=N, bm=x3, b_bs=Cn * N, b_ss=0,
              ldb=N, c=da, c_bs=Cn * Cn, ldc=Cn, precision=L.PREC_FP32)
    dgamma_c = K.dot(att, da)
    de = K.softmax_rows_bwd(att, da, -1.0)
    sym = K.add_transpose(de)
    K.conv_nn(B=B, M=Cn, Ck=Cn, ks=1, stride=1, pad=0, transposed=False, Hi=1, Wi=N, Ho=1, Wo=N, a=att,
              a_bs=Cn * Cn, a_sm=1, a_sc=Cn, a_st=0, x=d_cam, x_bs=d_bs, y=dx, y_bs=Cn * N,
              precision=prec, alpha=gamma_c, accumulate=True)
    K.conv_nn(B=B, M=Cn, Ck=Cn, ks=1, stride=1, pad=0, transposed=False, Hi=1, Wi=N, Ho=1, Wo=N, a=sym,
              a_bs=Cn * Cn, a_sm=Cn, a_sc=1, a_st=0, x=x3, x_bs=Cn * N, y=dx, y_bs=Cn * N,
              precision=prec, alpha=gamma_c, accumulate=True)
    return dgamma_c


class PamFn(Function):

    @staticmethod
    def forward(ctx, x, wq, bq, wk, bk, wv, bv, gamma_p):
        x = _c(x)
        prec = _prec("conv1x1")
        out = torch.empty_like(x)
        route, saved = _pam_forward(x, wq, bq, wk, bk, wv, bv, gamma_p, _as3(out), prec)
        ctx.save_for_backward(x, wq, wk, wv, gamma_p, *saved)
        ctx.cfg = (prec, route, (bq is not None, bk is not None, bv is not None))
        return out

    @staticmethod
    def backward(ctx, dout):
        x, wq, wk, wv, gamma_p, *saved = ctx.saved_tensors
        prec, route, has_bias = ctx.cfg
        B, Cn, H, W = x.shape
        d3 = _as3(_c(dout))
        dx = torch.empty(B, Cn, H * W, device=x.device, dtype=torch.float32)
        K.copy_slab(d3, dx)
        dwq, dbq, dwk, dbk, dwv, dbv, dg = _pam_backward(route, saved, x, wq, wk, wv, gamma_p, d3, dx, prec, has_bias)
        return dx.view(B, Cn, H, W), dwq, dbq, dwk, dbk, dwv, dbv, dg


class CamFn(Function):

    @staticmethod
    def forward(ctx, x, gamma_c):
        x = _c(x)
        out = torch.empty_like(x)
        ctx.prec = _prec("cam_apply")
        att = _cam_forward(x, gamma_c, _as3(out), ctx.prec)
        ctx.save_for_backward(x, gamma_c, att)
        return out

    @staticmethod
    def backward(ctx, dout):
        x, gamma_c, att = ctx.saved_tensors
        B, Cn, H, W = x.shape
        d3 = _as3(_c(dout))
        dx = torch.empty(B, Cn, H * W, device=x.device, dtype=torch.float32)
        K.copy_slab(d3, dx)
        dg = _cam_backward(att, x, gamma_c, d3, dx, ctx.prec)
        return dx.view(B, Cn, H, W), dg


class DualAttentionFn(Function):

    @staticmethod
    def forward(ctx, x, wq, bq, wk, bk, wv, bv, gamma_p, gamma_c):
        x = _c(x)
        B, Cn, H, W = x.shape
        prec, cprec = _prec("conv1x1"), _prec("cam_apply")
        feats = torch.empty(B, 2 * Cn, H, W, device=x.device, dtype=torch.float32)
        route, saved = _pam_forward(x, wq, bq, wk, bk, wv, bv, gamma_p, _as3(feats[:, :Cn]), prec)
        att = _cam_forward(x, gamma_c, _as3(feats[:, Cn:]), cprec)
        ctx.save_for_backward(x, wq, wk, wv, gamma_p, gamma_c, att, *saved)
        ctx.cfg = (prec, route, (bq is not None, bk is not None, bv is not None), cprec)
        return feats

    @staticmethod
    def backward(ctx, dfeat):
        x, wq, wk, wv, gamma_p, gamma_c, att, *saved = ctx.saved_tensors
        prec, route, has_bias, cprec = ctx.cfg
        B, Cn, H, W = x.shape
        dfeat = _c(dfeat)
        d_pam, d_cam = _as3(dfeat[:, :Cn]), _as3(dfeat[:, Cn:])
        dx = torch.empty(B, Cn, H * W, device=x.device, dtype=torch.float32)
        K.copy_slab(d_pam, dx)
        K.copy_slab(d_cam, dx, accumulate=True)
        dgc = _cam_backward(att, x, gamma_c, d_cam, dx, cprec)
        dwq, dbq, dwk, dbk, dwv, dbv, dgp = _pam_backward(route, saved, x, wq, wk, wv, gamma_p, d_pam, dx, prec, has_bias)
        return dx.view(B, Cn, H, W), dwq, dbq, dwk, dbk, dwv, dbv, dgp, dgc


def _as3(t: torch.Tensor) -> torch.Tensor:
    B, Cn, H, W = t.shape
    return t.as_strided((B, Cn, H * W), (t.stride(0), H * W, 1), t.storage_offset())


def _axpy_dev3(src: torch.Tensor, s: torch.Tensor, dst3: torch.Tensor) -> None:
    B = src.shape[0]
    if dst3.is_contiguous():
        K.scale_dev(src, s, out=dst3, accumulate=True)
        return
    for b in range(B):
        K.scale_dev(src[b], s, out=dst3[b], accumulate=True)


def _compact(t: torch.Tensor, rows: int, cols: int) -> torch.Tensor:
    B, Rp, Np = t.shape
    if Rp == rows and Np == cols:
        return t
    if Np == cols:
        return t[:, :rows]
    out = torch.empty(B, rows, cols, device=t.device, dtype=torch.float32)
    K.copy_rows(t, Rp * Np, Np, out, rows * cols, cols, B, rows, cols)
    return out


class BicubicFn(Function):
    @staticmethod
    def forward(ctx, x, Ho: int, Wo: int, rsh: float, rsw: float):
        x = _c(x)
        ctx.cfg = (x.shape[2], x.shape[3], rsh, rsw)
        return K.bicubic_fwd(x, Ho, Wo, rsh, rsw)

    @staticmethod
    def backward(ctx, dy):
        Hi, Wi, rsh, rsw = ctx.cfg
        return K.bicubic_bwd(_c(dy), Hi, Wi, rsh, rsw), None, None, None, None


def bicubic_up2(x):
    return BicubicFn.apply(x, 2 * x.shape[2], 2 * x.shape[3], 0.5, 0.5)


class BilinearFn(Function):
    @staticmethod
    def forward(ctx, x, Ho: int, Wo: int):
        x = _c(x)
        ctx.cfg = (x.shape[2], x.shape[3])
        return K.bilinear_fwd(x, Ho, Wo)

    @staticmethod
    def backward(ctx, dy):
        Hi, Wi = ctx.cfg
        return K.bilinear_bwd(_c(dy), Hi, Wi), None, None


class SkipFuseFn(Function):

    @staticmethod
    def forward(ctx, x, *wf):
        prec = _prec("conv1x1")
        n = len(wf) // 2
        ws, fs = wf[:n], [_c(f) for f in wf[n:]]
        x = _c(x)
        B, Co, Ho, Wo = x.shape
        s = K.conv2d_fwd(fs[0], ws[0], None, 1, 0, prec)
        for w, f in zip(ws[1:], fs[1:]):
            if f.shape[2:] != fs[0].shape[2:]:
                raise L.GandanetError("SkipFuseFn: all skip features must share one resolution")
            K.conv2d_fwd(f, w, None, 1, 0, prec, out=s, accumulate=True)
        out = K.bilinear_fwd(s, Ho, Wo, res=x)
        ctx.save_for_backward(*ws, *fs)
        ctx.cfg = (prec, n)
        return out

    @staticmethod
    def backward(ctx, dout):
        prec, n = ctx.cfg
        saved = ctx.saved_tensors
        ws, fs = saved[:n], saved[n:]
        dout = _c(dout)
# ... 393 lines not shown
```

include/gandanet.h:

```cpp
#ifndef GANDANET_H
#define GANDANET_H
#include <stddef.h>
#include <stdint.h>
#ifdef __cplusplus
extern "C" {
#endif

#define GD_VERSION 100
void gd_set_deterministic(int on);
int gd_get_deterministic(void);
int gd_set_det_reduce(int mode);
int gd_get_det_reduce(void);
int gd_version(void);
int gd_last_error(char* buf, int n);
int gd_sizeof_conv_desc(void);
int gd_sizeof_gemm_nt_desc(void);

enum { GD_PREC_FP32 = 0,
       GD_PREC_BF16 = 1,
       GD_PREC_X3 = 2     };
enum { GD_ACT_NONE = 0, GD_ACT_RELU = 1, GD_ACT_LEAKY02 = 2, GD_ACT_SIGMOID = 3 };

typedef struct gd_conv_desc {
    int B;
    int M;
    int Mstore;
    int Ck;
    int ks;
    int stride, pad;
    int transposed;
    int Hi, Wi;
    int Ho, Wo;
    const float* a; long a_bs, a_sm, a_sc, a_st;
    const float* x; long x_bs;
    const float* in_scale; const float* in_shift; int in_relu;
    void* y; long y_bs;
    int out_layout;
    int out_bf16;
    int ldo;
    const float* alpha; const float* bias; const float* res; long res_bs;
    int act; int accumulate;
    int precision;
    int sub_oy, sub_ox, sub_step;
} gd_conv_desc;
int gd_conv2d(const gd_conv_desc* d, void* stream);

size_t gd_conv3x3_ws_bytes(int M, int Ck);
int gd_conv3x3_eligible(const gd_conv_desc* d);
int gd_conv3x3(const gd_conv_desc* d, void* ws, size_t ws_bytes, void* stream);
int gd_conv3x3_wgrad(const float* dy, long dy_bs, const void* dy_bf16, const float* x, long x_bs, const void* x_nhwc16,
                     int x_ld, const float* in_scale, const float* in_shift, int in_relu, int B, int Cout, int Cin, int H,
                     int W, int stride, int accumulate, float* dw, void* stream);
int gd_conv3x3_wgrad_ws(const float* dy, long dy_bs, const void* dy_bf16, const float* x, long x_bs, const void* x_nhwc16,
                        int x_ld, const float* in_scale, const float* in_shift, int in_relu, int B, int Cout, int Cin, int H,
                        int W, int stride, int accumulate, float* dw, void* stream, void* ws, size_t ws_bytes);
int gd_conv3x3_wgrad_plan(int B, int Cout, int Cin, int H, int W, int stride, size_t ws_bytes, int* splits, size_t* ws_needed);

typedef struct gd_gemm_nt_desc {
    int B, M, N;
    int kseg; long klen;
    const float* a; long a_bs, a_ss, lda;
    const float* bm; long b_bs, b_ss, ldb;
    int im2col, ks, stride, pad, Hi, Wi, Ho, Wo;
    const float* in_scale; const float* in_shift; int in_relu;
    float* c; long c_bs, ldc;
    const float* alpha;
    const float* bias;
    int accumulate;
    int splits;
    int precision;
} gd_gemm_nt_desc;
int gd_gemm_nt(const gd_gemm_nt_desc* d, void* stream);
int gd_gemm_nt_ws(const gd_gemm_nt_desc* d, void* stream, void* ws, size_t ws_bytes);
int gd_gemm_nt_plan(const gd_gemm_nt_desc* d, size_t ws_bytes, int* splits, size_t* ws_needed);

size_t gd_bn_stats_ws_floats(int B, int C, long HW);
int gd_bn_stats(const float* x, long x_bs, int B, int C, long HW, float eps, float momentum,
                float* mean, float* invstd, float* running_mean, float* running_var, float* ws, void* stream);
int gd_bn_fold(const float* gamma, const float* beta, const float* mean, const float* invstd, int C,
               float* scale, float* shift, void* stream);
int gd_bn_stats_local(const float* x, long x_bs, int B, int C, long HW, float* stats, float* ws, void* stream);
int gd_bn_stats_merge(const float* stats_all, int world, int C, float eps, float momentum, float* mean, float* invstd,
                      float* running_mean, float* running_var, void* stream);
int gd_bn_act_bwd_dx(const float* dy, long dy_bs, const float* x, long x_bs, const float* scale, const float* shift,
                     const float* mean, const float* invstd, const float* dgamma_sum, const float* dbeta_sum, float inv_n,
                     int B, int C, long HW, int act, float* dx, long dx_bs, int accumulate_dx, void* stream);
int gd_bn_fold_eval(const float* gamma, const float* beta, const float* running_mean, const float* running_var,
                    float eps, int C, float* scale, float* shift, float* invstd_out, void* stream);
int gd_channel_sum(const float* x, long x_bs, int B, int C, long HW, float* out, int accumulate, float* ws,
                   void* stream);
int gd_affine_act(const float* x, long x_bs, const float* scale, const float* shift, int B, int C, long HW,
                  int act, float* y, long y_bs, void* stream);
int gd_bn_act_bwd(const float* dy, long dy_bs, const float* x, long x_bs, const float* scale, const float* shift,
                  const float* mean, const float* invstd, const float* gamma, int B, int C, long HW, int act,
                  int train, float* dgamma, float* dbeta, float* dx, long dx_bs, int accumulate_dx, float* ws,
                  void* stream);

int gd_bicubic_fwd(const float* x, int BC, int Hi, int Wi, float* y, int Ho, int Wo, float rscale_h,
                   float rscale_w, void* stream);
int gd_bicubic_bwd(const float* dy, int BC, int Hi, int Wi, float* dx, int Ho, int Wo, float rscale_h,
                   float rscale_w, void* stream);
int gd_shift_sum9_fwd(const float* u, const float* bias, float* y, int B, int H, int W, void* stream);
int gd_shift_sum9_bwd(const float* dy, float* du, int B, int H, int W, void* stream);
int gd_combine_inputs(const float* lr, int C1, int H1, int W1, float rs1, const float* aux, int C2, int H2, int W2,
                      float rs2, float* out, int B, int Ho, int Wo, void* stream);
int gd_bilinear_fwd(const float* x, int BC, int Hi, int Wi, float* y, int Ho, int Wo, int accumulate,
                    const float* res, void* stream);
int gd_bilinear_bwd(const float* dy, int BC, int Hi, int Wi, float* dx, int Ho, int Wo, void* stream);
int gd_maxpool2_fwd(const float* x, int BC, int Hi, int Wi, float* y, void* stream);
int gd_maxpool2_bwd(const float* x, const float* dy, int BC, int Hi, int Wi, float* dx, void* stream);

int gd_act_fwd(const float* x, float* y, long n, int act, void* stream);
int gd_act_bwd(const float* y, const float* dy, float* dx, long n, int act, void* stream);
int gd_axpby(const float* x, float a, float* y, float b, long n, void* stream);
int gd_scale_dev(const float* x, const float* s_dev, float* y, long n, int accumulate, void* stream);
int gd_copy_rows(const float* src, long s_bs, long s_ld, float* dst, long d_bs, long d_ld, int B, int R, int Cc,
                 void* stream);
int gd_copy_slab(const float* src, long s_bs, float* dst, long d_bs, int B, long chw, int accumulate, void* stream);
int gd_softmax_rows(const float* x, float* y, long rows, int cols, float sign, void* stream);
int gd_softmax_rows_bwd(const float* p, const float* dp, float* dx, long rows, int cols, float sign, void* stream);
int gd_dot(const float* a, const float* b, long n, float* out, int accumulate, float* ws, void* stream);
int gd_transpose(const float* s, float* t, int B, int R, int Cc, void* stream);
int gd_add_transpose(const float* a, float* out, int B, int n, void* stream);

int gd_bce_logits(const float* z, long n, float label, float* out, float* dz, float* ws, void* stream);
int gd_bce_logits_target(const float* z, const float* t, long n, float* out, float* dz, float* dt, float* ws,
                         void* stream);
int gd_leaky_fwd(const float* x, float* y, long n, float slope, void* stream);
// ... 19 lines not shown
                     void* y, int split, void* stream);
int gd_nhwc_stem_bwd(const void* g, int B, int Ci, int H, int W, const float* w, int Co, float* dimg, int split, void* stream);
int gd_nhwc_maxpool2_fwd(const void* x, int B, int H, int W, int C, void* y, int split, void* stream);
int gd_nhwc_maxpool2_bwd(const void* x, const void* dy, int B, int H, int W, int C, int relu_mask, void* dx, int split, void* stream);
int gd_nhwc_l1(const void* a, const void* b, long n, float* out, int accumulate, float* ws, int split_c, void* stream);
int gd_nhwc_l1_grad(const void* a, const void* b, long n, const float* upstream, int relu_mask, void* g, int split_c, void* stream);

int gd_disc_stem_fwd(const float* img, int B, int Ci, int H, int W, const float* w, const float* bias, int Co, float slope,
                     void* y, int split, void* stream);
int gd_disc_stem_wgrad(const void* g, const float* img, int B, int Ci, int H, int W, int Co, float* dw, float* db, int split, void* stream);
int gd_disc_stem_wgrad_ws(const void* g, const float* img, int B, int Ci, int H, int W, int Co, float* dw, float* db, int split,
                          void* stream, void* ws, size_t ws_bytes);
int gd_disc_stem_dgrad(const void* g, int B, int Ci, int H, int W, const float* w, int Co, float* dimg, int split, void* stream);
int gd_conv3x3_nhwc_s2(const void* x, const void* wpack, const float* bias, void* y, int B, int H, int W, int K, int M, int act,
                       float slope, int split, void* stream);
int gd_conv3x3_nhwc_s2_dgrad(const void* dy, const void* wpack_t, const void* act_out, float slope, void* dx, int B, int H,
                             int W, int K, int M, int split, void* stream);
int gd_nhwc_flatten_fwd(const void* y, int B, int HW, int C, float* f, int split, void* stream);
int gd_nhwc_flatten_bwd(const float* df, const void* y, float slope, int B, int HW, int C, void* g, int split, void* stream);
int gd_nhwc_to_nchw16(const void* g, int B, int HW, int C, void* gt, float* csum, int split, void* stream);
int gd_nhwc_to_nchw16_ws(const void* g, int B, int HW, int C, void* gt, float* csum, int split, void* stream, void* ws,
                         size_t ws_bytes);

int gd_pam_flash_fwd(const void* qt, const void* kt, const void* v, int B, int N, int Npad, int C, int Cp,
                     int v_ones, int f16, const float* gamma, const float* x, long x_bs, float* out, long out_bs,
                     float* o_attn, float* lse, const float* k_sqnorm_max, void* stream);
size_t gd_pam_fwd_shift_ws_bytes(int B, int Npad);
int gd_pam_flash_fwd_shift(const void* qt, const void* kt, const void* v, int B, int N, int Npad, int C, int Cp, int v_ones,
                           const float* gamma, const float* x, long x_bs, float* out, long out_bs, float* o_attn, float* lse,
                           int nsample, void* ws, size_t ws_bytes, void* stream);
int gd_pam_key_sqnorm_max(const void* kt, int B, int N, int Npad, int f16, float* out, void* stream);
#define GD_PAM_BWD_K64_ATOMIC 0
#define GD_PAM_BWD_K64_PARTS 1
#define GD_PAM_BWD_K32_PARTS 2
#define GD_PAM_BWD_TWO_KERNEL 3
size_t gd_pam_bwd_scratch_bytes(int Npad, int form);
int gd_pam_flash_bwd(const void* qt, const void* kt, const void* kn, const void* vt, const void* dot_,
                     const float* lse, const float* delta, int B, int N, int Npad, int Cp, int f16, int form,
                     float* dqn, float* dkn, float* dv, long out_bs, void* scratch, size_t scratch_bytes, void* stream);
int gd_pam_wide_fwd(const void* qt, const void* kt, const void* v, int B, int N, int Npad, int C, int Cp, int D, int f16,
                    const float* gamma, const float* x, long x_bs, float* out, long out_bs, float* o_attn, float* lse,
                    void* stream);
size_t gd_pam_wide_scratch_bytes(int Npad, int D, int deterministic);
int gd_pam_wide_bwd(const void* qt, const void* kt, const void* kn, const void* vt, const void* dot_, const float* lse,
                    const float* delta, int B, int N, int Npad, int Cp, int D, int f16, int deterministic, float* dqn,
                    float* dkn, float* dv, void* scratch, size_t scratch_bytes, void* stream);
int gd_pam_f32_fwd(const float* q, long q_bs, const float* k, long k_bs, const float* v, long v_bs, int B, int N, int Npad,
                   int C, int r, const float* gamma, const float* x, long x_bs, float* out, long out_bs, float* o_attn,
                   float* lse, void* stream);
int gd_pam_f32_bwd(const float* q, long q_bs, const float* k, long k_bs, const float* v, long v_bs, const float* gdo,
                   long gdo_bs, const float* lse, const float* delta, int B, int N, int Npad, int C, int r, float* dq,
                   float* dk, float* dv, void* stream);

int gd_pam_attn_stats(const float* q, long q_bs, const float* k, long k_bs, int B, int N, int Npad, int r, float logit_scale,
                      float* lse, float* entropy, float* peak, void* stream);
int gd_pam_attn_received(const float* q, long q_bs, const float* k, long k_bs, const float* lse, int B, int N, int Npad, int r,
                         float logit_scale, float* received, void* stream);
int gd_pam_attn_rows(const float* q, long q_bs, const float* k, long k_bs, const int* idx, int S, int B, int N, int Npad, int r,
                     float logit_scale, float* rows, float* lse_rows, void* stream);
int gd_round_to_16(const float* x, float* y, long n, float scale, int f16, void* stream);

size_t gd_hist_match_ws_bytes(long ns, long nt);
int gd_hist_match(const float* src, const float* ref, int B, long ns, long nt, double weight, double* out, void* ws,
                  size_t ws_bytes, void* stream);
int gd_blend_region(float* gen, const float* grace, const float* mask, int BC, int H, int W, int sr, int er, int sc,
                    int ec, void* stream);
int gd_augment_d4(const float* src, float* dst, int B, int C, int H, int W, const int* ops, const float* noise,
                  float noise_scale, void* stream);
int gd_bcast_mul(const float* x, const float* att, float* y, int B, int C, long HW, int mode, void* stream);
int gd_row_dot(const float* a, const float* b, float* out, long rows, long n, void* stream);
int gd_chan_maxmean_fwd(const float* x, float* y, int* idx, int B, int C, long HW, void* stream);
int gd_chan_maxmean_bwd(const float* dy, const int* idx, float* dx, int B, int C, long HW, void* stream);
int gd_chan_dot(const float* a, long a_bs, const float* o, long o_bs, int B, int C, int N, const float* gamma,
                float* d_raw, float* delta, void* stream);
int gd_pack_16_split(const float* s, long s_bs, int B, int R, int Cc, const float* row_scale, const float* row_shift, int relu,
                     void* plain, long p_bs, int ldp, long p_cs, int p_ncopy, int p_pattern, void* tr, long t_bs, int ldt,
                     long t_cs, int t_ncopy, int t_pattern, void* stream);
int gd_pack_16_split_masked(const float* s, long s_bs, int B, int R, int Cc, const float* row_scale, const float* row_shift,
                            int relu, void* plain, long p_bs, int ldp, long p_cs, int p_ncopy, int p_pattern, void* tr, long t_bs,
                            int ldt, long t_cs, int t_ncopy, int t_pattern, const float* mask, long m_bs, void* stream);
int gd_split3_weights(const float* w, long A, long Bn, long Cn, float* out, void* stream);
int gd_pam_f16_scale(const float* dout, long dout_bs, int B, int C, int N, const float* gamma, float* delta, float* scales,
                     float* ws, void* stream);
int gd_pack_bf16(const float* s, long s_bs, int B, int R, int Cc, const float* scale_dev, float scale_imm, void* plain,
                 int Rp_plain, int ld_plain, void* transposed, int Ccp_t, int ld_t, int perm16, int ones_row,
                 void* stream);
int gd_pack_16(const float* s, long s_bs, int B, int R, int Cc, const float* scale_dev, float scale_imm, void* plain,
               int Rp_plain, int ld_plain, void* transposed, int Ccp_t, int ld_t, int perm16, int ones_row, int f16,
               void* stream);
int gd_pack_16_affine(const float* s, long s_bs, int B, int R, int Cc, const float* row_scale, const float* row_shift, int relu,
                      void* plain, int Rp_plain, int ld_plain, void* transposed, int Ccp_t, int ld_t, int f16, void* stream);

int gd_comm_unique_id(char* id128);
int gd_comm_init(int rank, int world, const char* id128);
int gd_comm_world(void);
int gd_allreduce(void* buf, size_t n, int dtype, void* stream);
int gd_reduce_scatter(const void* send, void* recv, size_t recv_n, int dtype, void* stream);
int gd_allgather(const void* send, void* recv, size_t send_n, int dtype, void* stream);
int gd_comm_destroy(void);

enum { GD_EVAL_F64 = 1, GD_EVAL_SKIP_NAN = 2 };
size_t gd_eval_stats_ws_bytes(long n);
int gd_eval_stats(const void* pred, const void* truth, long planes, long hw, const unsigned char* mask, double a, double b,
                  int flags, double* rec, void* ws, size_t ws_bytes, void* stream);
size_t gd_masked_plane_mean_ws_bytes(long planes, long hw);
int gd_masked_plane_mean(const float* x, long planes, long hw, const unsigned char* mask, double* mean, long long* count,
                         void* ws, size_t ws_bytes, void* stream);
int gd_ensemble_stats(const void* x, int M, long member_stride, long n, int f64, void* mean, void* std_out, void* stream);
int gd_eval_merge_host(const double* recs, long k, double* rec_out, double* metrics);

enum { GD_GUARD_SQNORM = 0, GD_GUARD_NORM = 1, GD_GUARD_COEF = 2, GD_GUARD_OK = 3, GD_GUARD_APPLIED = 4, GD_GUARD_SKIPPED = 5,
       GD_GUARD_RECORD = 6 };
#define GD_GUARD_CHUNK 65536L
size_t gd_grad_sqnorm_ws_bytes(long total_chunks);
int gd_grad_sqnorm(const float* const* grads, const long* ns, int count, float gscale, int accumulate, double* rec, void* ws,
                   size_t ws_bytes, void* stream);
int gd_guard_finalize(double* rec, double max_norm, int skip_nonfinite, void* stream);
int gd_adamw_guarded(float* p, const float* g, float* m, float* v, float* ema, long n, const double* rec, float lr, float beta1,
                     float beta2, float eps, float weight_decay, float grad_scale, float ema_decay, void* stream);

enum { GD_FILTER_F32 = 0, GD_FILTER_F64 = 1 };
enum { GD_EDGE_REFLECT = 0, GD_EDGE_INTERIOR = 1 };
#define GD_FILTER_MAX_RADIUS 64
#define GD_SAVGOL_MAX_WINDOW 33
int gd_gaussian_weights_host(double sigma, double truncate, double* w, int cap);
int gd_correlate1d_axis(const void* src, void* dst, int dtype, long outer, long L, long inner, const double* w_host, int radius,
                        int edge_mode, void* stream);
int gd_savgol_edges_axis(const void* src, void* dst, int dtype, long outer, long L, long inner, const double* edge_dev,
                         int window, void* stream);
int gd_median_nd(const void* src, void* dst, int dtype, const int64_t* shape4, const int* size4, void* stream);
int gd_fill_prepare(const void* x, double placeholder, void* vals, void* mask, int dtype, long n, void* stream);
int gd_fill_ratio(const void* x, const void* num, const void* den, double placeholder, void* dst, int dtype, long n,
                  void* stream);

enum { GD_ZOOM_MIRROR = 0, GD_ZOOM_NEAREST = 1 };
size_t gd_zoom_axis_ws_bytes(long outer, long Lin, long inner, int order, int mode);
int gd_zoom_axis(const void* src, void* dst, int src_dtype, int dst_dtype, long outer, long Lin, long Lout, long inner,
                 int order, int mode, void* ws, size_t ws_bytes, void* stream);
int gd_spline_prefilter_axis(const void* src, double* dst, int src_dtype, long outer, long L, long inner, void* stream);
int gd_restore_units(const void* x, int x_dtype, const void* trend, int trend_dtype, const unsigned char* mask, long planes,
                     long hw, double scale, double mean, double unit, void* dst, int dst_dtype, void* stream);
size_t gd_masked_plane_mean_f64_ws_bytes(long planes, long hw);
int gd_masked_plane_mean_f64(const double* x, long planes, long hw, const unsigned char* mask, double* mean, long long* count,
                             void* ws, size_t ws_bytes, void* stream);

#define GD_FREQ_MAX_BINS 33
#define GD_FREQ_LDS_BYTES 32768
#define GD_FREQ_MAX_TABLE_BYTES (16L << 20)
size_t gd_channel_moments_ws_bytes(long M, long C);
int gd_channel_moments(const void* x, int dtype, long M, long C, double* rec, void* ws, size_t ws_bytes, void* stream);
int gd_scale_from_moments_host(const double* rec, long C, double* mean, double* var, double* scale);
int gd_channel_affine(const void* src, int src_dtype, void* dst, int dst_dtype, long M, long C, const double* mean_dev,
                      const double* scale_dev, int inverse, long N, long HW, void* stream);
int gd_freq_cos_table_host(long L, int K1, double* coef);
int gd_freq_augment_axis(const void* src, void* dst, int dtype, long outer, long L, long inner, const double* noise, int K1,
                         const double* coef, void* stream);

#define GD_ZONE_MAX 32
#define GD_ZONE_EDGE_CHUNK 512
int gd_zone_rasterize(const double* edges, long E, const long* edge_off, int Z, const double* xs, long W, const double* ys,
                      long H, unsigned int* bits, void* stream);
int gd_zone_rasterize_host(const double* edges, long E, const long* edge_off, int Z, const double* xs, long W,
                           const double* ys, long H, unsigned int* bits);
size_t gd_zone_mean_ws_bytes(long planes, long hw, int Z);
int gd_zone_mean(const void* x, int dtype, long planes, long hw, const unsigned int* bits, int Z, const double* weights,
                 double* mean, long long* count, void* ws, size_t ws_bytes, void* stream);
// ... 14 lines not shown
```

Baseline: 38.42 samples/s.

## Fuse PAM backward prologue, pair CAM 1x1 convs, exploit symmetric NT GEMM

Adds a fused PAM backward prologue kernel that computes the delta/dgamma reduction, the scaled 16-bit transposed dOut pack and the dx seed (d_pam + d_cam) in one pass, replacing separate chan_dot, scale, pack and copy launches. It also adds a paired 1x1 conv kernel that runs two accumulating GEMMs over the K dimension in a single launch for the CAM backward. A symmetric path in the NT GEMM skips lower-triangle tiles and mirrors them with an extra kernel. Weight concatenation moves to a single concat3_rows kernel. These cut launch count and redundant memory traffic, at the cost of more code paths and possible numeric ordering differences.

Result: no change. 38.66 samples/s (median of 6 runs) (+0.6%).

```diff
diff --git a/gan-danet_amd/_lib.py b/gan-danet_amd/_lib.py
--- a/gan-danet_amd/_lib.py
+++ b/gan-danet_amd/_lib.py
@@ -206,6 +206,10 @@
     "gd_allgather": (_i, [_p, _p, _sz, _i, _p]),
     "gd_comm_destroy": (_i, []),
     "gd_pack_bf16": (_i, [_p, _l, _i, _i, _i, _p, _f, _p, _i, _i, _p, _i, _i, _i, _i, _p]),
+    "gd_pam_bwd_prologue_ws_floats": (_sz, [_i, _i]),
+    "gd_pam_bwd_prologue": (_i, [_p, _l, _p, _l, _p, _l, _i, _i, _i, _i, _i, _p, _i, _p, _p, _p, _l, _p, _p, _p, _sz, _p]),
+    "gd_concat3_rows": (_i, [_p, _i, _i, _p, _i, _i, _p, _i, _i, _i, _i, _p, _p]),
+    "gd_conv1x1_pair": (_i, [C.POINTER(ConvDesc), _p, _l, _l, _l, _p, _l, _i, _p]),
     "gd_pack_16": (_i, [_p, _l, _i, _i, _i, _p, _f, _p, _i, _i, _p, _i, _i, _i, _i, _i, _p]),
     "gd_pack_16_affine": (_i, [_p, _l, _i, _i, _i, _p, _p, _i, _p, _i, _i, _p, _i, _i, _i, _p]),
 }
diff --git a/gan-danet_amd/csrc/gemm_conv.hip b/gan-danet_amd/csrc/gemm_conv.hip
--- a/gan-danet_amd/csrc/gemm_conv.hip
+++ b/gan-danet_amd/csrc/gemm_conv.hip
@@ -506,8 +506,9 @@
         }
 }
 
-template <int BM, bool X3 = false>
-__global__ __launch_bounds__(256) void conv1x1_tr_plain_kernel(const gd_conv_desc d) {
+struct conv_pair2 { const float* a; long a_bs, a_sm, a_sc; const float* x; long x_bs; int Ck; };
+template <int BM, bool X3 = false, bool PAIR = false>
+__global__ __launch_bounds__(256) void conv1x1_tr_plain_kernel(const gd_conv_desc d, const conv_pair2 p2) {
     constexpr int LDA = BK + 8;
     constexpr int A_PL = BM * LDA, X_PL = BK * XLD;
     constexpr int WAVES_N = gd::TileGeom<BM>::WAVES_N;
@@ -542,20 +543,32 @@
 
     float ra[KPT_A];
     float4 rx[4];
-    const int T = (d.Ck + BK - 1) / BK;
+    const int T1 = (d.Ck + BK - 1) / BK;
+    const int T = PAIR ? T1 + (p2.Ck + BK - 1) / BK : T1;
     auto load_tile = [&](int t) {
-        const int c0 = t * BK;
+        int c0 = t * BK, ck = d.Ck;
+        const float* ar = a_row;
+        const float* xi = x_img;
+        long asc = d.a_sc;
+        if constexpr (PAIR) {
+            if (t >= T1) {
+                c0 = (t - T1) * BK; ck = p2.Ck;
+                ar = p2.a + (long)b * p2.a_bs + (long)(m0 + am) * p2.a_sm;
+                xi = p2.x + (long)b * p2.x_bs;
+                asc = p2.a_sc;
+            }
+        }
 #pragma unroll
         for (int i = 0; i < KPT_A; ++i) {
             const int c = c0 + akg * KPT_A + i;
-            ra[i] = (a_row_ok && c < d.Ck) ? a_row[(long)c * d.a_sc] : 0.f;
+            ra[i] = (a_row_ok && c < ck) ? ar[(long)c * asc] : 0.f;
         }
 #pragma unroll
         for (int i = 0; i < 4; ++i) {
             const int c = c0 + xr0 + 8 * i;
             float4 v = make_float4(0.f, 0.f, 0.f, 0.f);
-            if (c < d.Ck) {
-                const float* p = x_img + (long)c * HW + pq;
+            if (c < ck) {
+                const float* p = xi + (long)c * HW + pq;
                 if (q_full) {
                     v = *reinterpret_cast<const float4*>(p);
                 } else {
@@ -785,13 +798,13 @@
         dim3 grid(gd_cdiv(HWl, BN * ns), gd_cdiv(d.M, bm), d.B);
 #define GD_C1X1(BM_, NS_) hipLaunchKernelGGL((conv1x1_tr_kernel<BM_, NS_>), grid, dim3(256), 0, s, d)
         if (d.precision == GD_PREC_X3) {
-            if (bm == 32) hipLaunchKernelGGL((conv1x1_tr_plain_kernel<32, true>), grid, dim3(256), 0, s, d);
-            else if (bm == 64) hipLaunchKernelGGL((conv1x1_tr_plain_kernel<64, true>), grid, dim3(256), 0, s, d);
-            else hipLaunchKernelGGL((conv1x1_tr_plain_kernel<128, true>), grid, dim3(256), 0, s, d);
+            if (bm == 32) hipLaunchKernelGGL((conv1x1_tr_plain_kernel<32, true>), grid, dim3(256), 0, s, d, conv_pair2{});
+            else if (bm == 64) hipLaunchKernelGGL((conv1x1_tr_plain_kernel<64, true>), grid, dim3(256), 0, s, d, conv_pair2{});
+            else hipLaunchKernelGGL((conv1x1_tr_plain_kernel<128, true>), grid, dim3(256), 0, s, d, conv_pair2{});
         } else if (ns == 1) {
-            if (bm == 32) hipLaunchKernelGGL((conv1x1_tr_plain_kernel<32>), grid, dim3(256), 0, s, d);
-            else if (bm == 64) hipLaunchKernelGGL((conv1x1_tr_plain_kernel<64>), grid, dim3(256), 0, s, d);
-            else hipLaunchKernelGGL((conv1x1_tr_plain_kernel<128>), grid, dim3(256), 0, s, d);
+            if (bm == 32) hipLaunchKernelGGL((conv1x1_tr_plain_kernel<32>), grid, dim3(256), 0, s, d, conv_pair2{});
+            else if (bm == 64) hipLaunchKernelGGL((conv1x1_tr_plain_kernel<64>), grid, dim3(256), 0, s, d, conv_pair2{});
+            else hipLaunchKernelGGL((conv1x1_tr_plain_kernel<128>), grid, dim3(256), 0, s, d, conv_pair2{});
         } else
         if (bm == 32) { if (ns == 4) GD_C1X1(32, 4); else if (ns == 2) GD_C1X1(32, 2); else GD_C1X1(32, 1); }
         else if (bm == 64) { if (ns == 4) GD_C1X1(64, 4); else if (ns == 2) GD_C1X1(64, 2); else GD_C1X1(64, 1); }
@@ -817,3 +830,39 @@
     }
     return run(d);
 }
+
+extern "C" int gd_conv1x1_pair(const gd_conv_desc* dp, const float* a2, long a2_bs, long a2_sm, long a2_sc, const float* x2,
+                               long x2_bs, int Ck2, void* stream) {
+    GD_CHECK_ARG(dp != nullptr && a2 && x2 && Ck2 > 0, "gd_conv1x1_pair: null descriptor or second pair");
+    gd_conv_desc d = *dp;
+    if (d.Mstore < d.M) d.Mstore = d.M;
+    GD_CHECK_ARG(d.ks == 1 && d.stride == 1 && d.pad == 0 && d.Hi == d.Ho && d.Wi == d.Wo && !d.in_scale && !d.in_shift &&
+                     d.act == GD_ACT_NONE && d.out_layout == 0 && !d.out_bf16 && d.Mstore == d.M && d.sub_step <= 1,
+                 "gd_conv1x1_pair: plain 1x1 convolutions into a channel-major fp32 output only");
+    static const int tr_env = getenv("GD_CONV1X1_TR") ? atoi(getenv("GD_CONV1X1_TR")) : 1;
+    if (tr_env && d.B > 0 && d.M > 0 && d.Ck > 0 && d.a && d.x && d.y && d.Ho > 0 && d.Wo > 0 && d.B <= 65535 &&
+        (long)d.Ho * d.Wo < (1L << 31) && conv1x1_tr_eligible(d) && x2_bs % 4 == 0 && ((uintptr_t)x2 % 16) == 0) {
+        const int bm = d.M <= 32 ? 32 : (d.M <= 64 || (d.M % 128 != 0 && d.M % 128 <= 64)) ? 64 : 128;
+        const conv_pair2 p2{a2, a2_bs, a2_sm, a2_sc, x2, x2_bs, Ck2};
+        hipStream_t s = (hipStream_t)stream;
+        dim3 grid(gd_cdiv((long)d.Ho * d.Wo, BN), gd_cdiv(d.M, bm), d.B);
+        if (d.precision == GD_PREC_X3) {
+            if (bm == 32) hipLaunchKernelGGL((conv1x1_tr_plain_kernel<32, true, true>), grid, dim3(256), 0, s, d, p2);
+            else if (bm == 64) hipLaunchKernelGGL((conv1x1_tr_plain_kernel<64, true, true>), grid, dim3(256), 0, s, d, p2);
+            else hipLaunchKernelGGL((conv1x1_tr_plain_kernel<128, true, true>), grid, dim3(256), 0, s, d, p2);
+        } else {
+            if (bm == 32) hipLaunchKernelGGL((conv1x1_tr_plain_kernel<32, false, true>), grid, dim3(256), 0, s, d, p2);
+            else if (bm == 64) hipLaunchKernelGGL((conv1x1_tr_plain_kernel<64, false, true>), grid, dim3(256), 0, s, d, p2);
+            else hipLaunchKernelGGL((conv1x1_tr_plain_kernel<128, false, true>), grid, dim3(256), 0, s, d, p2);
+        }
+        GD_LAUNCH_CHECK();
+        return 0;
+    }
+    int rc = gd_conv2d(&d, stream);
+    if (rc) return rc;
+    gd_conv_desc d2 = d;
+    d2.a = a2; d2.a_bs = a2_bs; d2.a_sm = a2_sm; d2.a_sc = a2_sc; d2.a_st = 0;
+    d2.x = x2; d2.x_bs = x2_bs; d2.Ck = Ck2;
+    d2.bias = nullptr; d2.res = nullptr; d2.res_bs = 0; d2.accumulate = 1;
+    return gd_conv2d(&d2, stream);
+}
diff --git a/gan-danet_amd/csrc/gemm_nt.hip b/gan-danet_amd/csrc/gemm_nt.hip
--- a/gan-danet_amd/csrc/gemm_nt.hip
+++ b/gan-danet_amd/csrc/gemm_nt.hip
@@ -20,9 +20,20 @@
     }
 }
 
+__global__ void mirror_lower_kernel(float* c, long c_bs, long ldc, int B, int M) {
+    const long total = (long)B * M * M;
+    for (long i = (long)blockIdx.x * blockDim.x + threadIdx.x; i < total; i += (long)gridDim.x * blockDim.x) {
+        const int n = (int)(i % M);
+        const long t = i / M;
+        const int m = (int)(t % M);
+        const int b = (int)(t / M);
+        if (m > n) c[(long)b * c_bs + (long)m * ldc + n] = c[(long)b * c_bs + (long)n * ldc + m];
+    }
+}
+
 template <int BM, int MODE, bool VEC = false>
 __global__ __launch_bounds__(256) void gemm_nt_kernel(const gd_gemm_nt_desc d, int ktiles, int tiles_per_split,
-                                                      int splits, float* part) {
+                                                      int splits, float* part, int sym) {
     constexpr bool BF16 = MODE != gd::MODE_F32;
     constexpr bool X3 = MODE == gd::MODE_X3;
     constexpr int A_PL = BM * gd::TilePol<MODE>::LD, B_PL = gd::TILE_BN * gd::TilePol<MODE>::LD;
@@ -46,6 +57,7 @@
     const int split = blockIdx.z - b * splits;
     const int m0 = blockIdx.y * BM;
     const int n0 = blockIdx.x * BN;
+    if (sym && m0 >= n0 + BN) return;
     const long K = (long)d.kseg * d.klen;
 
     const int kk = tid & 31;
@@ -283,6 +295,11 @@
     }
 }
 
+static bool nt_sym(const gd_gemm_nt_desc& d) {
+    return d.a == d.bm && d.a_bs == d.b_bs && d.a_ss == d.b_ss && d.lda == d.ldb && d.M == d.N && !d.im2col && !d.in_scale &&
+           !d.bias && !d.accumulate;
+}
+
 template <int BM>
 int launch(const gd_gemm_nt_desc& d, int ktiles, int tps, int splits, float* part, hipStream_t s) {
     if (splits > 1 && !d.accumulate && !part) {
@@ -291,21 +308,31 @@
         hipLaunchKernelGGL(fill_zero_kernel, dim3(blocks), dim3(256), 0, s, d.c, d.c_bs, d.ldc, d.B, d.M, d.N);
     }
     dim3 grid(gd_cdiv(d.N, BN), gd_cdiv(d.M, BM), d.B * splits);
+    const int sym = nt_sym(d);
     const bool vec = !d.im2col && d.klen % BK == 0 && d.lda % 4 == 0 && d.ldb % 4 == 0 &&
                      d.a_ss % 4 == 0 && d.b_ss % 4 == 0 && d.a_bs % 4 == 0 && d.b_bs % 4 == 0 &&
                      ((uintptr_t)d.a % 16) == 0 && ((uintptr_t)d.bm % 16) == 0;
     if (d.precision == GD_PREC_BF16) {
-        if (vec) hipLaunchKernelGGL((gemm_nt_kernel<BM, gd::MODE_BF16, true>), grid, dim3(256), 0, s, d, ktiles, tps, splits, part);
-        else hipLaunchKernelGGL((gemm_nt_kernel<BM, gd::MODE_BF16, false>), grid, dim3(256), 0, s, d, ktiles, tps, splits, part);
+        if (vec) hipLaunchKernelGGL((gemm_nt_kernel<BM, gd::MODE_BF16, true>), grid, dim3(256), 0, s, d, ktiles, tps, splits, part, sym);
+        else hipLaunchKernelGGL((gemm_nt_kernel<BM, gd::MODE_BF16, false>), grid, dim3(256), 0, s, d, ktiles, tps, splits, part, sym);
     } else if (d.precision == GD_PREC_X3) {
-        if (vec) hipLaunchKernelGGL((gemm_nt_kernel<BM, gd::MODE_X3, true>), grid, dim3(256), 0, s, d, ktiles, tps, splits, part);
-        else hipLaunchKernelGGL((gemm_nt_kernel<BM, gd::MODE_X3, false>), grid, dim3(256), 0, s, d, ktiles, tps, splits, part);
+        if (vec) hipLaunchKernelGGL((gemm_nt_kernel<BM, gd::MODE_X3, true>), grid, dim3(256), 0, s, d, ktiles, tps, splits, part, sym);
+        else hipLaunchKernelGGL((gemm_nt_kernel<BM, gd::MODE_X3, false>), grid, dim3(256), 0, s, d, ktiles, tps, splits, part, sym);
     } else {
-        if (vec) hipLaunchKernelGGL((gemm_nt_kernel<BM, gd::MODE_F32, true>), grid, dim3(256), 0, s, d, ktiles, tps, splits, part);
-        else hipLaunchKernelGGL((gemm_nt_kernel<BM, gd::MODE_F32, false>), grid, dim3(256), 0, s, d, ktiles, tps, splits, part);
+        if (vec) hipLaunchKernelGGL((gemm_nt_kernel<BM, gd::MODE_F32, true>), grid, dim3(256), 0, s, d, ktiles, tps, splits, part, sym);
+        else hipLaunchKernelGGL((gemm_nt_kernel<BM, gd::MODE_F32, false>), grid, dim3(256), 0, s, d, ktiles, tps, splits, part, sym);
     }
     GD_LAUNCH_CHECK();
-    if (part) return gd_det_reduce_launch(part, splits, d.c, d.B, d.M, d.N, d.c_bs, d.ldc, d.bias, d.accumulate, s);
+    if (part) {
+        const int rc = gd_det_reduce_launch(part, splits, d.c, d.B, d.M, d.N, d.c_bs, d.ldc, d.bias, d.accumulate, s);
+        if (rc) return rc;
+    }
+    if (sym) {
+        const long total = (long)d.B * d.M * d.M;
+        const int blocks = (int)((total + 255) / 256 > 4096 ? 4096 : (total + 255) / 256);
+        hipLaunchKernelGGL(mirror_lower_kernel, dim3(blocks), dim3(256), 0, s, d.c, d.c_bs, d.ldc, d.B, d.M);
+        GD_LAUNCH_CHECK();
+    }
     return 0;
 }
 
@@ -328,7 +355,12 @@
     const int bm = d.M <= 32 ? 32 : (d.M <= 64 || (d.M % 128 != 0 && d.M % 128 <= 64)) ? 64 : 128;
     int splits = d.splits;
     if (splits <= 0) {
-        const long tiles = (long)gd_cdiv(d.N, BN) * gd_cdiv(d.M, bm) * d.B;
+        long tiles = (long)gd_cdiv(d.N, BN) * gd_cdiv(d.M, bm) * d.B;
+        if (nt_sym(d)) {
+            tiles = 0;
+            for (int m0 = 0; m0 < d.M; m0 += bm)
+                for (int n0 = 0; n0 < d.N; n0 += BN) tiles += m0 < n0 + BN ? d.B : 0;
+        }
         splits = (int)(2048 / tiles);
         if (splits < 1) splits = 1;
         if (splits > ktiles / 8) splits = ktiles / 8 > 0 ? ktiles / 8 : 1;
diff --git a/gan-danet_amd/csrc/pointwise.hip b/gan-danet_amd/csrc/pointwise.hip
--- a/gan-danet_amd/csrc/pointwise.hip
+++ b/gan-danet_amd/csrc/pointwise.hip
@@ -483,6 +483,117 @@
     for (long i = (long)blockIdx.x * 256 + threadIdx.x; i < n; i += (long)gridDim.x * 256) delta[i] *= up;
 }
 
+template <bool VEC>
+__global__ __launch_bounds__(256) void pam_bwd_prologue_kernel(const float* __restrict__ dpam, long dp_bs,
+                                                              const float* __restrict__ oattn, long o_bs,
+                                                              const float* __restrict__ dcam, long dc_bs, int C, int N, int Np,
+                                                              int Cp, const float* __restrict__ scale, int f16, int fma_form,
+                                                              float* __restrict__ delta, unsigned short* __restrict__ tr,
+                                                              float* __restrict__ dx, long dx_bs, float* __restrict__ part) {
+    constexpr int TLD = 72;
+    __shared__ __attribute__((aligned(16))) unsigned short tile[64 * TLD];
+    __shared__ float red[16][64];
+    const int b = blockIdx.y, c0 = blockIdx.x * 64, tid = threadIdx.x;
+    const float k = *scale;
+    const float* dp = dpam + (long)b * dp_bs;
+    const float* op = oattn + (long)b * o_bs;
+    const float* cp = dcam ? dcam + (long)b * dc_bs : nullptr;
+    float* xp = dx ? dx + (long)b * dx_bs : nullptr;
+    auto cvt2 = [f16](float a, float bb) -> unsigned int {
+        if (f16) {
+            const unsigned int lo = __builtin_bit_cast(unsigned short, (_Float16)a), hi = __builtin_bit_cast(unsigned short, (_Float16)bb);
+            return lo | (hi << 16);
+        }
+        return gd_pack_bf2(a, bb);
+    };
+    auto ld4 = [N](const float* p, long off, int c) -> float4 {
+        if (VEC) return *reinterpret_cast<const float4*>(p + off);
+        float4 v = make_float4(0.f, 0.f, 0.f, 0.f);
+        v.x = p[off];
+        if (c + 1 < N) v.y = p[off + 1];
+        if (c + 2 < N) v.z = p[off + 2];
+        if (c + 3 < N) v.w = p[off + 3];
+        return v;
+    };
+    const int cg = (tid & 15) * 4, c = c0 + cg;
+    float4 acc = make_float4(0.f, 0.f, 0.f, 0.f);
+    for (int r0 = 0; r0 < Cp; r0 += 64) {
+#pragma unroll
+        for (int kk = 0; kk < 4; ++kk) {
+            const int rl = (tid >> 4) + 16 * kk, r = r0 + rl;
+            float4 v = make_float4(0.f, 0.f, 0.f, 0.f);
+            if (r < C && c < N) {
+                const long off = (long)r * N + c;
+                v = ld4(dp, off, c);
+                const float4 o = ld4(op, off, c);
+                acc.x = fmaf(v.x, o.x, acc.x); acc.y = fmaf(v.y, o.y, acc.y); acc.z = fmaf(v.z, o.z, acc.z); acc.w = fmaf(v.w, o.w, acc.w);
+                if (xp) {
+                    float4 w = v;
+                    if (cp) {
+                        const float4 q = ld4(cp, off, c);
+                        w.x = q.x + v.x; w.y = q.y + v.y; w.z = q.z + v.z; w.w = q.w + v.w;
+                    }
+                    if (VEC) {
+                        *reinterpret_cast<float4*>(xp + off) = w;
+                    } else {
+                        xp[off] = w.x;
+                        if (c + 1 < N) xp[off + 1] = w.y;
+                        if (c + 2 < N) xp[off + 2] = w.z;
+                        if (c + 3 < N) xp[off + 3] = w.w;
+                    }
+                }
+                if (fma_form) { v.x = fmaf(v.x, k, 0.f); v.y = fmaf(v.y, k, 0.f); v.z = fmaf(v.z, k, 0.f); v.w = fmaf(v.w, k, 0.f); }
+                else { v.x = k * v.x; v.y = k * v.y; v.z = k * v.z; v.w = k * v.w; }
+            }
+            uint2 w16;
+            w16.x = cvt2(v.x, v.y);
+            w16.y = cvt2(v.z, v.w);
+            *reinterpret_cast<uint2*>(tile + rl * TLD + cg) = w16;
+        }
+        __syncthreads();
+#pragma unroll
+        for (int kk = 0; kk < 2; ++kk) {
+            const int it = tid + 256 * kk;
+            const int cl = it >> 3, rg = (it & 7) * 8;
+            const int pc = c0 + cl, r = r0 + rg;
+            if (pc < Np && r < Cp) {
+                unsigned int w[4];
+#pragma unroll
+                for (int j = 0; j < 4; ++j)
+                    w[j] = (unsigned int)tile[(rg + 2 * j) * TLD + cl] | ((unsigned int)tile[(rg + 2 * j + 1) * TLD + cl] << 16);
+                *reinterpret_cast<uint4*>(tr + (long)b * Np * Cp + (long)pc * Cp + r) = make_uint4(w[0], w[1], w[2], w[3]);
+            }
+        }
+        __syncthreads();
+    }
+    red[tid >> 4][cg + 0] = acc.x;
+    red[tid >> 4][cg + 1] = acc.y;
+    red[tid >> 4][cg + 2] = acc.z;
+    red[tid >> 4][cg + 3] = acc.w;
+    __syncthreads();
+    if (tid < 64) {
+        float s = 0.f;
+#pragma unroll
+        for (int j = 0; j < 16; ++j) s += red[j][tid];
+        const int pc = c0 + tid;
+        if (pc < N) delta[(long)b * N + pc] = s * k;
+        else s = 0.f;
+        s = gd_wave_sum(s);
+        if (tid == 0) part[(long)b * gridDim.x + blockIdx.x] = s;
+    }
+}
+__global__ void concat3_rows_kernel(const float* __restrict__ s0, const float* __restrict__ s1, const float* __restrict__ s2,
+                                    int n0, int n1, int n2, int lo0, int lo1, int lo2, int cols, float* __restrict__ dst, long total) {
+    for (long i = (long)blockIdx.x * blockDim.x + threadIdx.x; i < total; i += (long)gridDim.x * blockDim.x) {
+        const int r = (int)(i / cols), cc = (int)(i - (long)r * cols);
+        float v = 0.f;
+        if (r >= lo0 && r < lo0 + n0) v = s0[(long)(r - lo0) * cols + cc];
+        else if (r >= lo1 && r < lo1 + n1) v = s1[(long)(r - lo1) * cols + cc];
+        else if (r >= lo2 && r < lo2 + n2) v = s2[(long)(r - lo2) * cols + cc];
+        dst[i] = v;
+    }
+}
+
 __global__ __launch_bounds__(256) void bce_kernel(const float* __restrict__ z, long n, float label, float inv_n,
                                                  float* __restrict__ dz, float* __restrict__ ws) {
     __shared__ float red[8];
@@ -932,6 +1043,57 @@
     return 0;
 }
 
+extern "C" size_t gd_pam_bwd_prologue_ws_floats(int B, int Np) { return (size_t)RED_BLOCKS + (size_t)B * gd_cdiv(Np, 64); }
+extern "C" int gd_pam_bwd_prologue(const float* d_pam, long dp_bs, const float* o_attn, long o_bs, const float* d_cam, long dc_bs,
+                                   int B, int C, int N, int Np, int Cp, const float* gamma, int f16, float* delta, void* dot16,
+                                   float* dx, long dx_bs, float* dgamma, float* scales, float* ws, size_t ws_floats,
+                                   void* stream) {
+    GD_CHECK_ARG(d_pam && o_attn && gamma && delta && dot16 && dgamma && ws && B > 0 && B <= 65535 && C > 0 && N > 0,
+                 "gd_pam_bwd_prologue: bad arguments");
+    GD_CHECK_ARG(Np >= N && Cp >= C && Cp % 8 == 0 && ((uintptr_t)dot16 % 16) == 0,
+                 "gd_pam_bwd_prologue: needs Np >= N, Cp >= C, Cp % 8 == 0 and a 16-byte aligned packed output");
+    GD_CHECK_ARG(!d_cam || dx, "gd_pam_bwd_prologue: d_cam without dx");
+    GD_CHECK_ARG(!f16 || scales, "gd_pam_bwd_prologue: the fp16 route needs the scales output");
+    GD_CHECK_ARG(dp_bs >= (long)C * N && o_bs >= (long)C * N && (!d_cam || dc_bs >= (long)C * N) && (!dx || dx_bs >= (long)C * N),
+                 "gd_pam_bwd_prologue: batch stride smaller than an image");
+    const int gx = gd_cdiv(Np, 64);
+    GD_CHECK_ARG(ws_floats >= gd_pam_bwd_prologue_ws_floats(B, Np), "gd_pam_bwd_prologue: workspace too small");
+    const float* scale = gamma;
+    if (f16) {
+        const long chw = (long)C * N;
+        int g = grid_for(chw);
+        g = g > RED_BLOCKS / B ? RED_BLOCKS / B : g;
+        g = g < 1 ? 1 : g;
+        GD_CHECK_ARG((long)g * B <= RED_BLOCKS, "gd_pam_bwd_prologue: batch larger than the reduction workspace (1024 parts)");
+        hipLaunchKernelGGL(absmax_kernel, dim3(g, B), dim3(256), 0, GD_S, d_pam, dp_bs, chw, ws);
+        hipLaunchKernelGGL(f16_scale_kernel, dim3(1), dim3(256), 0, GD_S, ws, g * B, gamma, (float*)nullptr, 0L, scales);
+        scale = scales;
+    }
+    auto al4 = [N](const float* p, long bs) { return !p || (N % 4 == 0 && bs % 4 == 0 && ((uintptr_t)p % 16) == 0); };
+    const int fma_form = al4(d_pam, dp_bs) ? 1 : 0;
+    const bool vec = fma_form && al4(o_attn, o_bs) && al4(d_cam, dc_bs) && al4(dx, dx_bs);
+    float* part = ws + RED_BLOCKS;
+    if (vec)
+        hipLaunchKernelGGL(pam_bwd_prologue_kernel<true>, dim3(gx, B), dim3(256), 0, GD_S, d_pam, dp_bs, o_attn, o_bs, d_cam, dc_bs,
+                           C, N, Np, Cp, scale, f16, fma_form, delta, (unsigned short*)dot16, dx, dx_bs, part);
+    else
+        hipLaunchKernelGGL(pam_bwd_prologue_kernel<false>, dim3(gx, B), dim3(256), 0, GD_S, d_pam, dp_bs, o_attn, o_bs, d_cam, dc_bs,
+                           C, N, Np, Cp, scale, f16, fma_form, delta, (unsigned short*)dot16, dx, dx_bs, part);
+    hipLaunchKernelGGL(reduce_final_kernel, dim3(1), dim3(256), 0, GD_S, part, gx * B, 1.f, dgamma, 0);
+    GD_LAUNCH_CHECK();
+    return 0;
+}
+extern "C" int gd_concat3_rows(const float* s0, int n0, int lo0, const float* s1, int n1, int lo1, const float* s2, int n2, int lo2,
+                               int R, int cols, float* dst, void* stream) {
+    GD_CHECK_ARG(s0 && s1 && s2 && dst && n0 > 0 && n1 > 0 && n2 > 0 && cols > 0, "gd_concat3_rows: bad arguments");
+    GD_CHECK_ARG(lo0 >= 0 && lo0 + n0 <= lo1 && lo1 + n1 <= lo2 && lo2 + n2 <= R, "gd_concat3_rows: row blocks must be ascending and disjoint");
+    const long total = (long)R * cols;
+    hipLaunchKernelGGL(concat3_rows_kernel, dim3(grid_for(total)), dim3(256), 0, GD_S, s0, s1, s2, n0, n1, n2, lo0, lo1, lo2, cols,
+                       dst, total);
+    GD_LAUNCH_CHECK();
+    return 0;
+}
+
 extern "C" int gd_bce_logits(const float* z, long n, float label, float* out, float* dz, float* ws, void* stream) {
     GD_CHECK_ARG(z && out && ws && n > 0, "gd_bce_logits: bad arguments");
     const int g = grid_for(n) > RED_BLOCKS ? RED_BLOCKS : grid_for(n);
diff --git a/gan-danet_amd/kern.py b/gan-danet_amd/kern.py
--- a/gan-danet_amd/kern.py
+++ b/gan-danet_amd/kern.py
@@ -115,7 +115,7 @@
             y: Tensor, y_bs: int, precision: int, Mstore: int = 0, in_scale: Optional[Tensor] = None,
             in_shift: Optional[Tensor] = None, in_relu: bool = False, out_layout: int = 0, out_bf16: bool = False,
             ldo: int = 0, alpha: Optional[Tensor] = None, bias: Optional[Tensor] = None,
-            res: Optional[Tensor] = None, res_bs: int = 0, act: int = 0, accumulate: bool = False) -> None:
+            res: Optional[Tensor] = None, res_bs: int = 0, act: int = 0, accumulate: bool = False, pair=None) -> None:
     d = L.ConvDesc()
     d.B, d.M, d.Mstore, d.Ck, d.ks, d.stride, d.pad = B, M, max(M, Mstore), Ck, ks, stride, pad
     d.transposed = int(transposed)
@@ -127,6 +127,11 @@
     d.out_layout, d.out_bf16, d.ldo = out_layout, int(out_bf16), ldo
     d.alpha, d.bias, d.res, d.res_bs = _ptr(alpha), _ptr(bias), _ptr(res), res_bs
     d.act, d.accumulate, d.precision = act, int(accumulate), precision
+    if pair is not None:
+        a2, a2_bs, a2_sm, a2_sc, x2, x2_bs, ck2 = pair
+        L.check(lib().gd_conv1x1_pair(C.byref(d), _ptr(a2), a2_bs, a2_sm, a2_sc, _ptr(x2), x2_bs, ck2, _stream()),
+                "gd_conv1x1_pair")
+        return
     if USE_CONV3X3_FAST and lib().gd_conv3x3_eligible(C.byref(d)):
         nbytes = int(lib().gd_conv3x3_ws_bytes(M, Ck))
         ws = torch.empty(nbytes // 2, device=x.device, dtype=torch.bfloat16)
@@ -725,6 +730,38 @@
     L.check(lib().gd_chan_dot(_ptr(a), abs_, _ptr(o), obs, B, Cn, N, _ptr(gamma), _ptr(d_raw), _ptr(delta), _stream()),
             "gd_chan_dot")
     return d_raw, delta
+
+
+def pam_bwd_prologue(d_pam: Tensor, o_attn: Tensor, gamma: Tensor, Np: int, Cp: int, *, d_cam: Optional[Tensor] = None,
+                     dx: Optional[Tensor] = None, f16: bool = False):
+    pbs, obs = _bview(d_pam, "dOut"), _bview(o_attn, "o_attn")
+    B, Cn = d_pam.shape[0], d_pam.shape[1]
+    N = d_pam[0, 0].numel()
+    dev = d_pam.device
+    delta = torch.empty(B, N, device=dev, dtype=torch.float32)
+    dgamma = torch.empty(1, device=dev, dtype=torch.float32)
+    dot16 = torch.empty(B, Np, Cp, device=dev, dtype=torch.float16 if f16 else torch.bfloat16)
+    scales = torch.empty(2, device=dev, dtype=torch.float32) if f16 else None
+    nws = int(lib().gd_pam_bwd_prologue_ws_floats(B, Np))
+    ws = torch.empty(nws, device=dev, dtype=torch.float32)
+    if d_cam is not None and d_cam.shape != d_pam.shape or dx is not None and dx.shape != d_pam.shape:
+        raise L.GandanetError("pam_bwd_prologue: d_cam / dx must have dOut's shape")
+    L.check(lib().gd_pam_bwd_prologue(_ptr(d_pam), pbs, _ptr(o_attn), obs, _ptr(d_cam), 0 if d_cam is None else _bview(d_cam),
+                                      B, Cn, N, Np, Cp, _ptr(gamma), int(f16), _ptr(delta), _ptr(dot16), _ptr(dx),
+                                      0 if dx is None else _bview(dx), _ptr(dgamma), _ptr(scales), _ptr(ws), nws, _stream()),
+            "gd_pam_bwd_prologue")
+    return delta, dgamma, dot16, scales
+
+
+def concat3_rows(srcs, los, R: int) -> Tensor:
+    ss = [_dense(s_, "concat source").reshape(s_.shape[0], -1) for s_ in srcs]
+    cols = ss[0].shape[1]
+    if len(ss) != 3 or any(s_.shape[1] != cols for s_ in ss):
+        raise L.GandanetError("concat3_rows: three sources with equal row length")
+    out = torch.empty(R, cols, device=ss[0].device, dtype=torch.float32)
+    L.check(lib().gd_concat3_rows(_ptr(ss[0]), ss[0].shape[0], los[0], _ptr(ss[1]), ss[1].shape[0], los[1], _ptr(ss[2]),
+                                  ss[2].shape[0], los[2], R, cols, _ptr(out), _stream()), "gd_concat3_rows")
+    return out
 
 
 def pam_f16_scale(dout: Tensor, gamma: Tensor, delta: Tensor) -> Tensor:
diff --git a/gan-danet_amd/ops.py b/gan-danet_amd/ops.py
--- a/gan-danet_amd/ops.py
+++ b/gan-danet_amd/ops.py
@@ -399,14 +399,10 @@
     x3 = x.view(B, Cn, N)
     route = _pam_route(B, Cn, r, N)
     if route != "chain" and PAM_CAT and (bq is None) == (bk is None) == (bv is None):
-        wc = torch.empty(2 * r + Cn, Cn, 1, 1, device=x.device, dtype=torch.float32)
-        for w_, lo in ((wq, 0), (wk, r), (wv, 2 * r)):
-            K.copy_slab(_c(w_).view(1, w_.shape[0], Cn), wc.view(1, 2 * r + Cn, Cn)[:, lo:lo + w_.shape[0]])
+        wc = K.concat3_rows((_c(wq), _c(wk), _c(wv)), (0, r, 2 * r), 2 * r + Cn).view(2 * r + Cn, Cn, 1, 1)
         bc = None
         if bq is not None:
-            bc = torch.empty(2 * r + Cn, device=x.device, dtype=torch.float32)
-            for b_, lo in ((bq, 0), (bk, r), (bv, 2 * r)):
-                K.copy_slab(b_.view(1, -1, 1), bc.view(1, -1, 1)[:, lo:lo + b_.numel()])
+            bc = K.concat3_rows((_c(bq), _c(bk), _c(bv)), (0, r, 2 * r), 2 * r + Cn).view(2 * r + Cn)
         y3 = K.conv2d_fwd(x, wc, bc, 1, 0, prec).view(B, 2 * r + Cn, N)
         q, k, v = y3[:, :r], y3[:, r:2 * r], y3[:, 2 * r:]
     else:
@@ -485,7 +481,19 @@
     return K.transpose(dqt), K.transpose(dkt), dv, dgamma_p
 
 
-def _pam_backward(route, pam_saved, x, wq, wk, wv, gamma_p, d_pam, dx, prec, has_bias):
+def _pam_bwd_seed(route, pam_saved, x, gamma_p, d_pam, d_cam, dx):
+    if route in ("narrow", "wide"):
+        qt, o_attn = pam_saved[0], pam_saved[4]
+        N = x.shape[2] * x.shape[3]
+        return K.pam_bwd_prologue(d_pam, o_attn, gamma_p, _npad(N), _cp(x.shape[1]), d_cam=d_cam, dx=dx,
+                                  f16=qt.dtype == torch.float16)
+    K.copy_slab(d_pam, dx)
+    if d_cam is not None:
+        K.copy_slab(d_cam, dx, accumulate=True)
+    return None
+
+
+def _pam_backward(route, pam_saved, x, wq, wk, wv, gamma_p, d_pam, dx, prec, has_bias, pro=None):
     B, Cn, H, W = x.shape
     N = H * W
     r = wq.shape[0]
@@ -507,14 +515,9 @@
     elif route in ("narrow", "wide"):
         qt, kt, kn, vt, o_attn, lse = pam_saved
         Np, Cp = _npad(N), _cp(Cn)
-        d_raw, delta = K.chan_dot(d_pam, o_attn, gamma_p)
-        dgamma_p = K.dot(d_raw, None)
         f16 = qt.dtype == torch.float16
-        s_up, s_inv = gamma_p, None
-        if f16:
-            scales = K.pam_f16_scale(d_pam, gamma_p, delta)
-            s_up, s_inv = scales[0:1], scales[1:2]
-        _, dot_ = K.pack_bf16(d_pam, Cn, N, scale=s_up, t_shape=(Np, Cp), f16=f16)
+        delta, dgamma_p, dot_, scales = pro
+        s_inv = scales[1:2] if f16 else None
         if route == "wide":
             D = qt.shape[2]
             dqn = torch.empty(B, D, Np, device=x.device, dtype=torch.float32)
@@ -526,9 +529,7 @@
             dcat = torch.empty(B, R, Np, device=x.device, dtype=torch.float32)
             K.pam_flash_bwd(qt, kt, kn, vt, dot_, lse, delta, B, N, Np, Cp, dcat[:, 0:32], dcat[:, 32:64], dcat[:, 64:],
                             r_alg=r, c_alg=Cn, f16=f16, out_bs=R * Np)
-            wcat = torch.zeros(R, Cn, 1, 1, device=x.device, dtype=torch.float32)
-            for w_, lo in ((wq, 0), (wk, 32), (wv, 64)):
-                K.copy_slab(_c(w_).view(1, w_.shape[0], Cn), wcat.view(1, R, Cn)[:, lo:lo + w_.shape[0]])
+            wcat = K.concat3_rows((_c(wq), _c(wk), _c(wv)), (0, 32, 64), R).view(R, Cn, 1, 1)
             dcat4 = dcat.view(B, R, H, W)
             dwc = K.conv2d_wgrad(dcat4, x, 1, 1, 0, prec, alpha=s_inv)
             dbc = K.channel_sum(dcat4) if any(has_bias) else None
@@ -589,10 +590,7 @@
     sym = K.add_transpose(de)
     K.conv_nn(B=B, M=Cn, Ck=Cn, ks=1, stride=1, pad=0, transposed=False, Hi=1, Wi=N, Ho=1, Wo=N, a=att,
               a_bs=Cn * Cn, a_sm=1, a_sc=Cn, a_st=0, x=d_cam, x_bs=d_bs, y=dx, y_bs=Cn * N,
-              precision=prec, alpha=gamma_c, accumulate=True)
-    K.conv_nn(B=B, M=Cn, Ck=Cn, ks=1, stride=1, pad=0, transposed=False, Hi=1, Wi=N, Ho=1, Wo=N, a=sym,
-              a_bs=Cn * Cn, a_sm=Cn, a_sc=1, a_st=0, x=x3, x_bs=Cn * N, y=dx, y_bs=Cn * N,
-              precision=prec, alpha=gamma_c, accumulate=True)
+              precision=prec, alpha=gamma_c, accumulate=True, pair=(sym, Cn * Cn, Cn, 1, x3, Cn * N, Cn))
     return dgamma_c
 
 
@@ -615,8 +613,8 @@
         B, Cn, H, W = x.shape
         d3 = _as3(_c(dout))
         dx = torch.empty(B, Cn, H * W, device=x.device, dtype=torch.float32)
-        K.copy_slab(d3, dx)
-        dwq, dbq, dwk, dbk, dwv, dbv, dg = _pam_backward(route, saved, x, wq, wk, wv, gamma_p, d3, dx, prec, has_bias)
+        pro = _pam_bwd_seed(route, saved, x, gamma_p, d3, None, dx)
+        dwq, dbq, dwk, dbk, dwv, dbv, dg = _pam_backward(route, saved, x, wq, wk, wv, gamma_p, d3, dx, prec, has_bias, pro)
         return dx.view(B, Cn, H, W), dwq, dbq, dwk, dbk, dwv, dbv, dg
 
 
@@ -664,10 +662,9 @@
         dfeat = _c(dfeat)
         d_pam, d_cam = _as3(dfeat[:, :Cn]), _as3(dfeat[:, Cn:])
         dx = torch.empty(B, Cn, H * W, device=x.device, dtype=torch.float32)
-        K.copy_slab(d_pam, dx)
-        K.copy_slab(d_cam, dx, accumulate=True)
+        pro = _pam_bwd_seed(route, saved, x, gamma_p, d_pam, d_cam, dx)
         dgc = _cam_backward(att, x, gamma_c, d_cam, dx, cprec)
-        dwq, dbq, dwk, dbk, dwv, dbv, dgp = _pam_backward(route, saved, x, wq, wk, wv, gamma_p, d_pam, dx, prec, has_bias)
+        dwq, dbq, dwk, dbk, dwv, dbv, dgp = _pam_backward(route, saved, x, wq, wk, wv, gamma_p, d_pam, dx, prec, has_bias, pro)
         return dx.view(B, Cn, H, W), dwq, dbq, dwk, dbk, dwv, dbv, dgp, dgc
 
 
diff --git a/include/gandanet.h b/include/gandanet.h
--- a/include/gandanet.h
+++ b/include/gandanet.h
@@ -44,6 +44,8 @@
     int sub_oy, sub_ox, sub_step;
 } gd_conv_desc;
 int gd_conv2d(const gd_conv_desc* d, void* stream);
+int gd_conv1x1_pair(const gd_conv_desc* d, const float* a2, long a2_bs, long a2_sm, long a2_sc, const float* x2, long x2_bs,
+                    int Ck2, void* stream);
 
 size_t gd_conv3x3_ws_bytes(int M, int Ck);
 int gd_conv3x3_eligible(const gd_conv_desc* d);
@@ -229,6 +231,12 @@
 int gd_split3_weights(const float* w, long A, long Bn, long Cn, float* out, void* stream);
 int gd_pam_f16_scale(const float* dout, long dout_bs, int B, int C, int N, const float* gamma, float* delta, float* scales,
                      float* ws, void* stream);
+size_t gd_pam_bwd_prologue_ws_floats(int B, int Np);
+int gd_pam_bwd_prologue(const float* d_pam, long dp_bs, const float* o_attn, long o_bs, const float* d_cam, long dc_bs, int B,
+                        int C, int N, int Np, int Cp, const float* gamma, int f16, float* delta, void* dot16, float* dx,
+                        long dx_bs, float* dgamma, float* scales, float* ws, size_t ws_floats, void* stream);
+int gd_concat3_rows(const float* s0, int n0, int lo0, const float* s1, int n1, int lo1, const float* s2, int n2, int lo2, int R,
+                    int cols, float* dst, void* stream);
 int gd_pack_bf16(const float* s, long s_bs, int B, int R, int Cc, const float* scale_dev, float scale_imm, void* plain,
                  int Rp_plain, int ld_plain, void* transposed, int Ccp_t, int ld_t, int perm16, int ones_row,
                  void* stream);
```
